# mcgillmrl/prob_mbrl

Hardware: AMD Instinct MI355X
Metric: particle_rollouts_per_sec (higher is better)
Workload: dtype f32 via split fp16 (fwd, 2 pieces) / bf16 (adjoint, 2 pieces) MFMA, fp32 accumulate

## Files before the change

include/pmbrl.h:

```cpp
#ifndef PMBRL_H
#define PMBRL_H

#include <stddef.h>
#include <stdint.h>

#ifdef __cplusplus
extern "C" {
#endif

#define PMBRL_MAX_LAYERS 8
#define PMBRL_MAX_ANGLE 8
#define PMBRL_MAX_TIP 8
#define PMBRL_MAX_DIM 64

#define PMBRL_FLAG_MM_STATES 1
#define PMBRL_FLAG_MM_REWARDS 2
#define PMBRL_FLAG_INFER_NS 4
#define PMBRL_FLAG_FORCE_GENERIC 16
#define PMBRL_FLAG_NO_SHAPED 32
#define PMBRL_FLAG_POL_MASKS_PER_STEP 64
#define PMBRL_FLAG_DYN_MASKS_PER_STEP 128
#define PMBRL_FLAG_GMM_EXACT_NOISE_GRAD 256
#define PMBRL_MAX_COMP 8
#define PMBRL_FLAG_ZMM_PER_STEP 8
// ... 28 lines not shown
  int32_t expand;
  int32_t n_angle;
  int32_t angle_dims[PMBRL_MAX_ANGLE];
  int32_t k;
  float C[PMBRL_MAX_TIP * PMBRL_MAX_DIM];
  float tip_target[PMBRL_MAX_TIP];
  float norm;
  float w;
  float Q[PMBRL_MAX_TIP * PMBRL_MAX_TIP];
  float R[PMBRL_MAX_DIM * PMBRL_MAX_DIM];
} pmbrl_reward;

typedef struct pmbrl_config {
  int32_t B, D, U, H;
  int32_t B_global, row_offset;
  int32_t flags;
  int32_t mm_groups;
  float max_log_std_pol;
  float max_log_std_dyn;
  pmbrl_mlp pol;
  pmbrl_mlp dyn;
  pmbrl_reward reward;
  int32_t rows_per_wg_hint;
  int32_t precision;
  int32_t n_pol_angle;
  int32_t pol_angle_dims[PMBRL_MAX_ANGLE];
  int32_t n_dyn_angle;
  int32_t dyn_angle_dims[PMBRL_MAX_ANGLE];
  int32_t dyn_components;
  int32_t mm_span_rows, mm_span_offset;
  int32_t mm_span_ranks, mm_span_rank;
  int32_t pol_act, dyn_act;
} pmbrl_config;


typedef struct pmbrl_plan pmbrl_plan;

enum {
  PMBRL_INFO_ROWS_PER_WG = 0,
  PMBRL_INFO_N_WG = 1,
  PMBRL_INFO_ROW_TILES = 2,
  PMBRL_INFO_LDS_BYTES = 3,
  PMBRL_INFO_N_POL_PARAMS = 4,
  PMBRL_INFO_N_DYN_PARAMS = 5,
  PMBRL_INFO_DW_SPLITS = 6,
  PMBRL_INFO_MM_MODE = 7,
  PMBRL_INFO_LD = 8,
  PMBRL_INFO_DW_BLOCKS = 9,
  PMBRL_INFO_FAST = 10,
  PMBRL_INFO_STAGES = 11,
  PMBRL_INFO_MM_GRID = 12,
  PMBRL_INFO_PRECISION = 13,
  PMBRL_INFO_DW_PIPE = 14,
  PMBRL_INFO_MM_PARTS = 15,
  PMBRL_INFO_REG = 16,
  PMBRL_INFO_REPLAY = 17,
  PMBRL_INFO_INPLACE = 18,
  PMBRL_INFO_REG_FWD_CALLS = 19,
  PMBRL_INFO_REG_BWD_CALLS = 20,
  PMBRL_INFO_TAIL_CALLS = 21,
  PMBRL_INFO_COUNT = 22
};

const char* pmbrl_last_error(void);
int pmbrl_act_check(int32_t act, int32_t n_hidden);
int pmbrl_version(void);
const char* pmbrl_build_id(void);

typedef struct pmbrl_graph pmbrl_graph;
int pmbrl_graph_capture_begin(void* stream);
int pmbrl_graph_capture_end(void* stream, pmbrl_graph** graph_out);
int pmbrl_graph_launch(pmbrl_graph* graph, void* stream);
int pmbrl_graph_num_nodes(pmbrl_graph* graph, int64_t* n_out);
void pmbrl_graph_destroy(pmbrl_graph* graph);

int pmbrl_plan_create(const pmbrl_config* cfg, int device, pmbrl_plan** out);
void pmbrl_plan_destroy(pmbrl_plan* plan);
size_t pmbrl_plan_workspace_bytes(const pmbrl_plan* plan);
int pmbrl_plan_info(const pmbrl_plan* plan, int32_t* info );
#define PMBRL_SWEEP_REG 4
int pmbrl_plan_sweep_kernel(const pmbrl_plan* plan, int variant, int adjoint, const char** name);
int pmbrl_plan_dw_stream(const pmbrl_plan* plan, int32_t* out );
int pmbrl_plan_dw_head(const pmbrl_plan* plan);

int pmbrl_pack_mask(void* stream, const float* mask_d, int32_t B, int32_t h,
                    int32_t src_ld, uint16_t* bits_d);

int pmbrl_draw_masks(void* stream, int32_t kind, uint64_t seed, uint64_t offset, const float* param_d,
                     int32_t param_len, float temp, int32_t rows, int32_t h, const float* u_d, const float* v_d,
                     uint16_t* bits_d, int32_t aux_row0, int32_t aux_rows, float* u_out_d, float* hard_out_d,
                     float* probs_out_d);

typedef struct pmbrl_inputs {
  const float* x0_d;
  const float* pol_params_d;
  const float* dyn_params_d;
  const float* mx_d;
  const float* iSx_d;
  const float* my_d;
  const float* Sy_d;
  const float* pol_scale_d;
  const float* pol_bias_d;
  const uint16_t* pol_mask_bits_d[PMBRL_MAX_LAYERS];
  const uint16_t* dyn_mask_bits_d[PMBRL_MAX_LAYERS];
  const float* z_pol_d;
  const float* z_dyn_d;
  int64_t z_pol_step_stride;
  int64_t z_dyn_step_stride;
  const float* z_mm_d;
  const float* z_rr_d;
  const float* z_pi_d;
  const float* u_cat_d;
} pmbrl_inputs;

int pmbrl_rollout_fwd(pmbrl_plan* plan, void* stream, void* workspace_d,
                      const pmbrl_inputs* in, float* states_d, float* actions_d,
                      float* rewards_d, int32_t* status_d);

int pmbrl_rollout_bwd(pmbrl_plan* plan, void* stream, void* workspace_d,
                      const pmbrl_inputs* in, const float* states_d,
                      const float* actions_d, const float* rewards_d,
                      const float* grad_rewards_d, const float* grad_states_d,
                      const float* grad_actions_d, float* grad_pol_flat_d,
                      float* grad_x0_d, float* action_grad_norms_d, int32_t* status_d);

int pmbrl_weighted_sum(void* stream, const float* a_d, const float* w_d,
                       int64_t n, float* out_d);
int pmbrl_weighted_sum_steps(void* stream, const float* a_d, const float* w_d,
                             int64_t n_per_step, int32_t n_steps, const int32_t* status_d,
                             float* out_d);

int pmbrl_clip_adam(void* stream, float* params_d, float* grads_d,
                    float* exp_avg_d, float* exp_avg_sq_d, int64_t n,
                    int64_t step, double lr, double beta1, double beta2, double eps,
                    double max_norm, float* norm_out_d);

int pmbrl_clip_adam_guarded(void* stream, float* params_d, float* grads_d,
                            float* exp_avg_d, float* exp_avg_sq_d, int64_t n,
                            int64_t* step_d, double lr, double beta1, double beta2,
                            double eps, double max_norm, float* norm_out_d,
                            const int32_t* status_d, int32_t expect);

typedef struct pmbrl_adam {
  float* params_d;
  float* exp_avg_d;
  float* exp_avg_sq_d;
  int64_t* step_d;
  double lr, beta1, beta2, eps, max_norm;
  float* norm_out_d;
  int32_t expect_steps;
  float* loss_out_d;
} pmbrl_adam;
int pmbrl_plan_set_loss(pmbrl_plan* plan, const float* loss_weights_d, float* loss_out_d);
int pmbrl_rollout_bwd_adam(pmbrl_plan* plan, void* stream, void* workspace_d, const pmbrl_inputs* in,
                           const float* states_d, const float* actions_d, const float* rewards_d,
                           const float* grad_rewards_d, const float* grad_states_d, const float* grad_actions_d,
                           float* grad_pol_flat_d, float* grad_x0_d, float* action_grad_norms_d, int32_t* status_d,
                           const pmbrl_adam* opt);

#define PMBRL_OPT_MAX_GROUPS   8
#define PMBRL_OPT_MAX_SEGMENTS 32
#define PMBRL_OPT_DECOUPLED 1
#define PMBRL_OPT_AMSGRAD   2
#define PMBRL_OPT_MAXIMIZE  4
typedef struct pmbrl_opt_group { double lr, beta1, beta2, eps, weight_decay; int32_t flags; } pmbrl_opt_group;
typedef struct pmbrl_opt_rule {
// ... 148 lines not shown
```

prob_mbrl_amd/_lib.py:

```python
import ctypes as C
import os

_HERE = os.path.dirname(os.path.abspath(__file__))
LIB_PATH = os.environ.get('PMBRL_LIB_PATH', os.path.join(_HERE, 'csrc', 'libpmbrl_hip.so'))

MAX_LAYERS = 8
MAX_ANGLE = 8
MAX_TIP = 8
MAX_DIM = 64
FLAG_MM_STATES, FLAG_MM_REWARDS, FLAG_INFER_NS, FLAG_ZMM_PER_STEP = 1, 2, 4, 8
FLAG_FORCE_GENERIC = 16
FLAG_NO_SHAPED = 32
FLAG_POL_MASKS_PER_STEP, FLAG_DYN_MASKS_PER_STEP = 64, 128
FLAG_GMM_EXACT_NOISE_GRAD = 256
MAX_COMP = 8
REWARD_EXP, REWARD_NEG, REWARD_LEARNED = 0, 1, 2
PREC_F32, PREC_SPLIT, PREC_SPLIT_F16 = 0, 1, 2
ACT_RELU, ACT_TANH, ACT_SILU = 0, 1, 2
DROP_BY_TEMPERATURE, DROP_BERNOULLI = 0, 1
MLP_BWD_MAX_BLOCKS = 256
MLP_BWD_SLAB_BYTES = 64 << 20
(INFO_ROWS_PER_WG, INFO_N_WG, INFO_ROW_TILES, INFO_LDS_BYTES, INFO_N_POL_PARAMS, INFO_N_DYN_PARAMS, INFO_DW_SPLITS,
 INFO_MM_MODE, INFO_LD, INFO_DW_BLOCKS, INFO_FAST, INFO_STAGES, INFO_MM_GRID, INFO_PRECISION, INFO_DW_PIPE, INFO_MM_PARTS,
 INFO_REG, INFO_REPLAY, INFO_INPLACE, INFO_REG_FWD_CALLS, INFO_REG_BWD_CALLS, INFO_TAIL_CALLS, INFO_COUNT) = range(23)
SWEEP_VARIANTS = ('lean', 'ext', 'mm', 'mmg', 'reg')
TIMER_COUNT = 8
TIMER_NAMES = ['pack', 'fwd', 'bwd', 'dw', 'dw_reduce', 'reward']


class MLP(C.Structure):
    _fields_ = [('n_layers', C.c_int32),
                ('dims', C.c_int32 * (MAX_LAYERS + 1)),
                ('keep', C.c_float * MAX_LAYERS)]


class MlpCall(C.Structure):
    _fields_ = [('B', C.c_int32), ('net', MLP), ('max_log_std', C.c_float), ('act', C.c_int32)]


class BnnConfig(C.Structure):
    _fields_ = [('M', C.c_int32), ('N', C.c_int32), ('net', MLP), ('max_log_std', C.c_float),
                ('temperature', C.c_float * MAX_LAYERS), ('reg_scale', C.c_float * MAX_LAYERS),
                ('drop_reg', C.c_float * MAX_LAYERS), ('reg_weight', C.c_float), ('loss_kind', C.c_int32),
                ('n_components', C.c_int32), ('act', C.c_int32),
                ('drop_kind', C.c_int32 * MAX_LAYERS), ('bern_keep', C.c_float * MAX_LAYERS)]


class Reward(C.Structure):
    _fields_ = [('kind', C.c_int32), ('expand', C.c_int32),
                ('n_angle', C.c_int32), ('angle_dims', C.c_int32 * MAX_ANGLE),
                ('k', C.c_int32), ('C', C.c_float * (MAX_TIP * MAX_DIM)),
                ('tip_target', C.c_float * MAX_TIP), ('norm', C.c_float),
                ('w', C.c_float), ('Q', C.c_float * (MAX_TIP * MAX_TIP)),
                ('R', C.c_float * (MAX_DIM * MAX_DIM))]


class Config(C.Structure):
    _fields_ = [('B', C.c_int32), ('D', C.c_int32), ('U', C.c_int32),
                ('H', C.c_int32), ('B_global', C.c_int32),
                ('row_offset', C.c_int32), ('flags', C.c_int32),
                ('mm_groups', C.c_int32), ('max_log_std_pol', C.c_float),
                ('max_log_std_dyn', C.c_float), ('pol', MLP), ('dyn', MLP),
                ('reward', Reward), ('rows_per_wg_hint', C.c_int32), ('precision', C.c_int32),
                ('n_pol_angle', C.c_int32), ('pol_angle_dims', C.c_int32 * MAX_ANGLE),
                ('n_dyn_angle', C.c_int32), ('dyn_angle_dims', C.c_int32 * MAX_ANGLE),
                ('dyn_components', C.c_int32),
                ('mm_span_rows', C.c_int32), ('mm_span_offset', C.c_int32),
                ('mm_span_ranks', C.c_int32), ('mm_span_rank', C.c_int32),
                ('pol_act', C.c_int32), ('dyn_act', C.c_int32)]


COLLECTIVE_FN = C.CFUNCTYPE(C.c_int, C.c_void_p, C.c_void_p, C.c_void_p, C.c_int64)


class Inputs(C.Structure):
    _fields_ = [('x0', C.c_void_p), ('pol_params', C.c_void_p),
                ('dyn_params', C.c_void_p), ('mx', C.c_void_p),
                ('iSx', C.c_void_p), ('my', C.c_void_p), ('Sy', C.c_void_p),
                ('pol_scale', C.c_void_p), ('pol_bias', C.c_void_p),
                ('pol_mask_bits', C.c_void_p * MAX_LAYERS),
                ('dyn_mask_bits', C.c_void_p * MAX_LAYERS),
                ('z_pol', C.c_void_p), ('z_dyn', C.c_void_p),
                ('z_pol_step_stride', C.c_int64), ('z_dyn_step_stride', C.c_int64),
                ('z_mm', C.c_void_p), ('z_rr', C.c_void_p),
                ('z_pi', C.c_void_p), ('u_cat', C.c_void_p)]


EXPORTS = [
    'pmbrl_last_error', 'pmbrl_version', 'pmbrl_build_id', 'pmbrl_plan_create',
    'pmbrl_graph_capture_begin', 'pmbrl_graph_capture_end', 'pmbrl_graph_launch', 'pmbrl_graph_num_nodes', 'pmbrl_graph_destroy',
    'pmbrl_plan_destroy', 'pmbrl_plan_workspace_bytes', 'pmbrl_plan_info', 'pmbrl_plan_sweep_kernel', 'pmbrl_plan_dw_stream',
    'pmbrl_plan_dw_head',
    'pmbrl_pack_mask', 'pmbrl_draw_masks', 'pmbrl_rollout_fwd', 'pmbrl_rollout_bwd', 'pmbrl_rollout_bwd_adam',
    'pmbrl_plan_set_loss',
    'pmbrl_weighted_sum', 'pmbrl_weighted_sum_steps', 'pmbrl_clip_adam', 'pmbrl_clip_adam_guarded', 'pmbrl_debug_linear',
    'pmbrl_plan_set_timing', 'pmbrl_plan_read_timing', 'pmbrl_plan_set_prof', 'pmbrl_plan_set_replay', 'pmbrl_plan_replay_count',
    'pmbrl_mlp_workspace_bytes', 'pmbrl_mlp_forward', 'pmbrl_mlp_grad_input',
    'pmbrl_mlp_backward_workspace_bytes', 'pmbrl_mlp_backward',
    'pmbrl_bnn_plan_create', 'pmbrl_bnn_plan_destroy', 'pmbrl_bnn_plan_workspace_bytes',
    'pmbrl_bnn_plan_n_params', 'pmbrl_bnn_plan_set_unit_keep', 'pmbrl_bnn_loss_grad', 'pmbrl_bnn_loss_grad_ex', 'pmbrl_bnn_train_steps',
    'pmbrl_comm_unique_id', 'pmbrl_comm_init', 'pmbrl_allreduce_sum', 'pmbrl_comm_count', 'pmbrl_comm_destroy',
    'pmbrl_plan_set_comm', 'pmbrl_plan_set_collective',
    'pmbrl_p2p_create', 'pmbrl_p2p_handle', 'pmbrl_p2p_open', 'pmbrl_p2p_allreduce_f32', 'pmbrl_p2p_allreduce_f64',
    'pmbrl_plan_set_p2p', 'pmbrl_p2p_error', 'pmbrl_p2p_destroy', 'pmbrl_plan_set_grad_comm',
    'pmbrl_opt_rule_check', 'pmbrl_clip_adam_rule', 'pmbrl_clip_adam_rule_guarded', 'pmbrl_plan_set_optimizer',
    'pmbrl_bnn_plan_set_optimizer', 'pmbrl_act_check',
]

class Adam(C.Structure):
    _fields_ = [('params_d', C.c_void_p), ('exp_avg_d', C.c_void_p), ('exp_avg_sq_d', C.c_void_p),
                ('step_d', C.c_void_p), ('lr', C.c_double), ('beta1', C.c_double), ('beta2', C.c_double),
                ('eps', C.c_double), ('max_norm', C.c_double), ('norm_out_d', C.c_void_p), ('expect_steps', C.c_int32),
                ('loss_out_d', C.c_void_p)]


OPT_MAX_GROUPS, OPT_MAX_SEGMENTS = 8, 32
OPT_DECOUPLED, OPT_AMSGRAD, OPT_MAXIMIZE = 1, 2, 4


class OptGroup(C.Structure):
    _fields_ = [('lr', C.c_double), ('beta1', C.c_double), ('beta2', C.c_double), ('eps', C.c_double),
                ('weight_decay', C.c_double), ('flags', C.c_int32)]


class OptRule(C.Structure):
    _fields_ = [('n_groups', C.c_int32), ('group', OptGroup * OPT_MAX_GROUPS),
                ('n_segments', C.c_int32), ('seg_end', C.c_int64 * OPT_MAX_SEGMENTS),
                ('seg_group', C.c_int32 * OPT_MAX_SEGMENTS), ('max_exp_avg_sq_d', C.c_void_p)]


_lib = None


def load():
    global _lib
    if _lib is not None:
        return _lib
    if not os.path.exists(LIB_PATH):
        raise RuntimeError(
            'prob_mbrl_amd: %s is missing -- build the HIP extension first '
            '(python -c "import __graft_entry__ as g; g.build()"). There is no '
            'CPU fallback for the rollout hot path.' % LIB_PATH)
    lib = C.CDLL(LIB_PATH)
    vp, i32, i64, f32 = C.c_void_p, C.c_int32, C.c_int64, C.c_float
    lib.pmbrl_last_error.restype = C.c_char_p
    lib.pmbrl_last_error.argtypes = []
    lib.pmbrl_version.restype = C.c_int
    lib.pmbrl_build_id.restype = C.c_char_p
    lib.pmbrl_build_id.argtypes = []
    lib.pmbrl_graph_capture_begin.restype = C.c_int
    lib.pmbrl_graph_capture_begin.argtypes = [vp]
    lib.pmbrl_graph_capture_end.restype = C.c_int
    lib.pmbrl_graph_capture_end.argtypes = [vp, C.POINTER(vp)]
    lib.pmbrl_graph_launch.restype = C.c_int
    lib.pmbrl_graph_launch.argtypes = [vp, vp]
    lib.pmbrl_graph_num_nodes.restype = C.c_int
    lib.pmbrl_graph_num_nodes.argtypes = [vp, C.POINTER(C.c_int64)]
    lib.pmbrl_graph_destroy.restype = None
    lib.pmbrl_graph_destroy.argtypes = [vp]
    lib.pmbrl_plan_create.restype = C.c_int
    lib.pmbrl_plan_create.argtypes = [C.POINTER(Config), C.c_int, C.POINTER(vp)]
    lib.pmbrl_plan_destroy.restype = None
    lib.pmbrl_plan_destroy.argtypes = [vp]
    lib.pmbrl_plan_workspace_bytes.restype = C.c_size_t
    lib.pmbrl_plan_workspace_bytes.argtypes = [vp]
    lib.pmbrl_plan_info.restype = C.c_int
    lib.pmbrl_plan_info.argtypes = [vp, C.POINTER(i32)]
    lib.pmbrl_plan_sweep_kernel.restype = C.c_int
    lib.pmbrl_plan_sweep_kernel.argtypes = [vp, C.c_int, C.c_int, C.POINTER(C.c_char_p)]
    if hasattr(lib, 'pmbrl_plan_dw_stream'):
        lib.pmbrl_plan_dw_stream.restype = C.c_int
        lib.pmbrl_plan_dw_stream.argtypes = [vp, C.POINTER(i32)]
    if hasattr(lib, 'pmbrl_plan_dw_head'):
        lib.pmbrl_plan_dw_head.restype = C.c_int
        lib.pmbrl_plan_dw_head.argtypes = [vp]
    lib.pmbrl_pack_mask.restype = C.c_int
    lib.pmbrl_pack_mask.argtypes = [vp, vp, i32, i32, i32, vp]
    lib.pmbrl_rollout_fwd.restype = C.c_int
    lib.pmbrl_rollout_fwd.argtypes = [vp, vp, vp, C.POINTER(Inputs), vp, vp, vp, vp]
    lib.pmbrl_rollout_bwd.restype = C.c_int
    lib.pmbrl_rollout_bwd.argtypes = [vp, vp, vp, C.POINTER(Inputs), vp, vp, vp,
                                      vp, vp, vp, vp, vp, vp, vp]
    lib.pmbrl_weighted_sum.restype = C.c_int
    lib.pmbrl_weighted_sum.argtypes = [vp, vp, vp, i64, vp]
    lib.pmbrl_weighted_sum_steps.restype = C.c_int
    lib.pmbrl_weighted_sum_steps.argtypes = [vp, vp, vp, i64, i32, vp, vp]
    lib.pmbrl_clip_adam.restype = C.c_int
    f64 = C.c_double
    lib.pmbrl_clip_adam.argtypes = [vp, vp, vp, vp, vp, i64, i64, f64, f64, f64,
                                    f64, f64, vp]
    lib.pmbrl_clip_adam_guarded.restype = C.c_int
    lib.pmbrl_clip_adam_guarded.argtypes = [vp, vp, vp, vp, vp, i64, vp, f64, f64, f64, f64, f64, vp, vp, i32]
    lib.pmbrl_mlp_workspace_bytes.restype = C.c_size_t
    lib.pmbrl_mlp_workspace_bytes.argtypes = [C.POINTER(MlpCall)]
    lib.pmbrl_mlp_forward.restype = C.c_int
    lib.pmbrl_mlp_forward.argtypes = [vp, C.POINTER(MlpCall), vp, vp, vp, C.POINTER(vp)] + [vp] * 10
    lib.pmbrl_mlp_grad_input.restype = C.c_int
    lib.pmbrl_mlp_grad_input.argtypes = [vp, C.POINTER(MlpCall), vp, vp, vp, C.POINTER(vp)] + [vp] * 11
    lib.pmbrl_mlp_backward_workspace_bytes.restype = C.c_size_t
    lib.pmbrl_mlp_backward_workspace_bytes.argtypes = [C.POINTER(MlpCall)]
    lib.pmbrl_mlp_backward.restype = C.c_int
    lib.pmbrl_mlp_backward.argtypes = [vp, C.POINTER(MlpCall), vp, vp, vp, C.POINTER(vp)] + [vp] * 12
    lib.pmbrl_bnn_plan_create.restype = C.c_int
    lib.pmbrl_bnn_plan_create.argtypes = [C.POINTER(BnnConfig), C.c_int, C.POINTER(vp)]
    lib.pmbrl_bnn_plan_destroy.restype = None
    lib.pmbrl_bnn_plan_destroy.argtypes = [vp]
    lib.pmbrl_bnn_plan_workspace_bytes.restype = C.c_size_t
    lib.pmbrl_bnn_plan_workspace_bytes.argtypes = [vp]
    lib.pmbrl_bnn_plan_n_params.restype = C.c_int64
    lib.pmbrl_bnn_plan_n_params.argtypes = [vp]
    lib.pmbrl_bnn_plan_set_unit_keep.restype = C.c_int
    lib.pmbrl_bnn_plan_set_unit_keep.argtypes = [vp, i32, C.POINTER(f32), i32]
    lib.pmbrl_bnn_loss_grad.restype = C.c_int
    lib.pmbrl_bnn_loss_grad.argtypes = [vp] * 11
    lib.pmbrl_bnn_loss_grad_ex.restype = C.c_int
    lib.pmbrl_bnn_loss_grad_ex.argtypes = [vp] * 13 + [i32]
    lib.pmbrl_bnn_train_steps.restype = C.c_int
    lib.pmbrl_bnn_train_steps.argtypes = ([vp] * 6 + [i32] + [vp] * 4 + [C.c_double] * 4 + [C.c_uint64] * 2 + [vp] * 4)
    lib.pmbrl_debug_linear.restype = C.c_int
    lib.pmbrl_debug_linear.argtypes = [vp, vp, vp, vp, i32, i32, i32, i32, vp, vp]
    lib.pmbrl_plan_set_replay.restype = C.c_int
    lib.pmbrl_plan_set_replay.argtypes = [vp, C.c_int]
    lib.pmbrl_plan_replay_count.restype = C.c_int
    lib.pmbrl_plan_replay_count.argtypes = [vp, C.POINTER(C.c_int64)]
    lib.pmbrl_plan_set_timing.restype = C.c_int
    lib.pmbrl_plan_set_timing.argtypes = [vp, C.c_int]
    lib.pmbrl_plan_read_timing.restype = C.c_int
    lib.pmbrl_plan_read_timing.argtypes = [vp, C.POINTER(C.c_float)]
    lib.pmbrl_plan_set_prof.restype = C.c_int
    lib.pmbrl_plan_set_prof.argtypes = [vp, vp, vp]
    lib.pmbrl_comm_unique_id.restype = C.c_int
    lib.pmbrl_comm_unique_id.argtypes = [vp]
    lib.pmbrl_comm_init.restype = C.c_int
    lib.pmbrl_comm_init.argtypes = [vp, i32, i32, i32, C.POINTER(vp)]
    lib.pmbrl_allreduce_sum.restype = C.c_int
    lib.pmbrl_allreduce_sum.argtypes = [vp, vp, vp, i64]
    lib.pmbrl_plan_set_loss.restype = C.c_int
    lib.pmbrl_plan_set_loss.argtypes = [vp, vp, vp]
    lib.pmbrl_rollout_bwd_adam.restype = C.c_int
    lib.pmbrl_rollout_bwd_adam.argtypes = [vp, vp, vp, C.POINTER(Inputs)] + [vp] * 10 + [C.POINTER(Adam)]
    lib.pmbrl_draw_masks.restype = C.c_int
    lib.pmbrl_draw_masks.argtypes = [vp, i32, C.c_uint64, C.c_uint64, vp, i32, C.c_float, i32, i32, vp, vp, vp, i32, i32, vp, vp, vp]
    lib.pmbrl_comm_count.restype = C.c_int
    lib.pmbrl_comm_count.argtypes = [vp, C.POINTER(i32)]
    lib.pmbrl_comm_destroy.restype = None
    lib.pmbrl_comm_destroy.argtypes = [vp]
    lib.pmbrl_plan_set_comm.restype = C.c_int
    lib.pmbrl_plan_set_comm.argtypes = [vp, vp]
    lib.pmbrl_p2p_create.restype = C.c_int
    lib.pmbrl_p2p_create.argtypes = [i32, i32, i32, i64, C.POINTER(vp)]
    lib.pmbrl_p2p_handle.restype = C.c_int
    lib.pmbrl_p2p_handle.argtypes = [vp, vp]
    lib.pmbrl_p2p_open.restype = C.c_int
    lib.pmbrl_p2p_open.argtypes = [vp, i32, vp]
    for fn in (lib.pmbrl_p2p_allreduce_f32, lib.pmbrl_p2p_allreduce_f64):
        fn.restype = C.c_int
        fn.argtypes = [vp, vp, vp, i64]
    lib.pmbrl_plan_set_p2p.restype = C.c_int
# ... 39 lines not shown
```

prob_mbrl_amd/csrc/pmbrl.hip:

```cpp
#include <hip/hip_runtime.h>
#include <math.h>
#include <stdio.h>
#include <string.h>

#include <algorithm>
#include <memory>
#include <string>
#include <vector>

#include "pmbrl_host.h"
#include "pmbrl_mm.h"
#include "pmbrl_rollout.h"
#include "pmbrl_mmx.h"
#include "pmbrl_mm_wide.h"
#include "pmbrl_fast.h"
#include "pmbrl_reward.h"

static thread_local std::string g_err;
int pm_fail(int code, const std::string& msg) {
  g_err = msg;
  return code;
}

extern "C" const char* pmbrl_last_error(void) { return g_err.c_str(); }
// ... 293 lines not shown
  return why ? fail(-2, why) : 0;
}

static int net_plan(const pmbrl_mlp& m, int act, NetPlan& n, int in_expect, int out_expect,
                    const char* name) {
  if (m.n_layers < 1 || m.n_layers > PM_MAXL)
    return fail(-2, std::string(name) + ": n_layers out of range");
  n.nl = m.n_layers;
  size_t off = 0;
  for (int i = 0; i <= n.nl; ++i) {
    if (m.dims[i] < 1 || m.dims[i] > 4096) return fail(-2, std::string(name) + ": bad layer width");
    n.dim[i] = m.dims[i];
    n.nt[i] = (m.dims[i] + 15) / 16;
  }
  if (n.dim[0] != in_expect || n.dim[n.nl] != out_expect)
    return fail(-2, std::string(name) + ": input/output width does not match D/U");
  if (const char* why = pm_act_refusal(act, n.nl - 1)) return fail(-2, std::string(name) + ": " + why);
  n.act = pm_act_layers(act, n.nl - 1);
  for (int l = 0; l < n.nl; ++l) {
    n.keep[l] = (l < n.nl - 1) ? m.keep[l] : 1.f;
    if (l < n.nl - 1 && !(n.keep[l] > 0.f)) return fail(-2, std::string(name) + ": keep must be > 0");
    n.w_off[l] = off;
    off += (size_t)n.dim[l + 1] * n.dim[l];
    n.b_off[l] = off;
    off += n.dim[l + 1];
  }
  n.n_params = off;
  return 0;
}

#define PM_INST(RT, CA, CB, VAR, D, U, LD, NL, NT, TREE) \
  {reinterpret_cast<const void*>(&pm_rollout_fwd<RT>), reinterpret_cast<const void*>(&pm_rollout_bwd<RT>)},
static const PmInst general_f32_fns[] = {PM_GENERAL_F32_INSTANCES};
#undef PM_INST
static_assert(sizeof(general_f32_fns) / sizeof(general_f32_fns[0]) == pm_general_f32_n, "one kernel pair per key");

static constexpr size_t PM_LDS_CAP = 160 * 1024;

static bool env_set(const char* name) { return getenv(name) != nullptr; }
static bool env_on(const char* name) {
  const char* e = getenv(name);
  return !(e && atoi(e) == 0);
}
static PlanSwitches read_switches() {
  PlanSwitches s{};
  s.mm_perstep = env_set("PMBRL_MM_PERSTEP");
  s.mm_mode2 = env_set("PMBRL_MM_MODE2");
  s.mm_no_batch = env_set("PMBRL_MM_NO_BATCH");
  s.dw_no_wide = env_set("PMBRL_DW_NO_WIDE");
  s.reg_debug = env_set("PMBRL_REG_DEBUG");
  s.lds_tiles = env_on("PMBRL_LDS_TILES");
  s.mm_xch = env_on("PMBRL_MM_XCH");
  s.mm_tree = env_on("PMBRL_MM_TREE");
  s.reg = env_on("PMBRL_REG");
  s.reg_mm = env_on("PMBRL_REG_MM");
  s.reg_tree = env_on("PMBRL_REG_TREE");
  s.reg_bwd = env_on("PMBRL_REG_BWD");
  s.fuse_loss = env_on("PMBRL_FUSE_LOSS");
  s.ztab_merge = env_on("PMBRL_ZTAB_MERGE");
  s.wide = env_on("PMBRL_WIDE");
  if (const char* e = getenv("PMBRL_MM_PARTS")) { s.mm_parts_set = true; s.mm_parts = atoi(e); }
  s.replay = 1;
  if (const char* e = getenv("PMBRL_REPLAY")) s.replay = std::max(0, std::min(2, atoi(e)));
  if (const char* e = getenv("PMBRL_DW_PIPE")) {
    s.dw_pipe_off = !strcmp(e, "off");
    s.dw_pipe_ranges = e[0] >= '0' && e[0] <= '9';
    for (const char* q = e; s.dw_pipe_ranges && *q;) {
      const int v = atoi(q);
      if (v > 0) s.dw_pipe.push_back(v);
      while (*q && *q != ',') ++q;
      if (*q == ',') ++q;
    }
  }
  s.dw_head = -1;
  if (const char* e = getenv("PMBRL_DW_HEAD")) s.dw_head = !strcmp(e, "on") ? 1 : (!strcmp(e, "off") ? 0 : -1);
  if (const char* e = getenv("PMBRL_DW_STREAM")) {
    s.dw_stream_off = !strcmp(e, "off");
    s.dw_stream_set = e[0] >= '0' && e[0] <= '9';
    if (s.dw_stream_set) {
      s.dw_stream_steps = atoi(e);
      if (const char* q = strchr(e, ',')) s.dw_stream_wgs = std::max(0, atoi(q + 1));
    }
  }
  return s;
}

static int plan_nets(pmbrl_plan* p) {
  const pmbrl_config& c = p->cfg;
  if (c.n_pol_angle < 0 || c.n_pol_angle > PMBRL_MAX_ANGLE || c.n_dyn_angle < 0 || c.n_dyn_angle > PMBRL_MAX_ANGLE)
    return fail(-2, "n_pol_angle / n_dyn_angle out of range");
  if (c.dyn_components < 0 || c.dyn_components > PMBRL_MAX_COMP)
    return fail(-2, "dyn_components out of range (<= PMBRL_MAX_COMP)");
  const bool gmm = c.dyn_components > 1;
  if (c.reward.kind != PMBRL_REWARD_EXP && c.reward.kind != PMBRL_REWARD_NEG && c.reward.kind != PMBRL_REWARD_LEARNED)
    return fail(-2, "unknown reward kind");
  p->learned = c.reward.kind == PMBRL_REWARD_LEARNED;
  if (p->learned && c.mm_span_rows > 0)
    return fail(-2, "learned reward head: not offered with moment-matching groups spread over ranks (mm_span_rows > 0)");
  if (p->learned && c.D + 1 > PMBRL_MAX_DIM) return fail(-2, "learned reward head: D + 1 exceeds PMBRL_MAX_DIM");
  if (p->learned && gmm && c.dyn.n_layers >= 1 && c.dyn.n_layers <= PM_MAXL &&
      c.dyn.dims[c.dyn.n_layers] != (2 * (c.D + 1) + 1) * c.dyn_components + 1)
    return fail(-2, "learned reward head with the mixture head: the density has D + 1 dimensions, a dynamics head "
                    "(2 (D + 1) + 1) dyn_components + 1 wide");
  int rc = net_plan(c.pol, c.pol_act, p->pol, c.D + c.n_pol_angle, 2 * c.U, "policy");
  if (rc == 0)
    rc = net_plan(c.dyn, c.dyn_act, p->dyn, c.D + c.U + c.n_dyn_angle,
                  gmm ? (2 * (c.D + p->learned) + 1) * c.dyn_components + 1 : 2 * (c.D + p->learned), "dynamics");
  p->act = rc == 0 && (p->pol.act != 0 || p->dyn.act != 0);
  return rc;
}

struct LayoutCalc {
  const pmbrl_plan* p;
  int maxnt;
  bool gsplit;
  bool want_split;
  bool rt4_split;
  int ld_generic() const { return gsplit ? (maxnt * 16 + 31) / 32 * 32 + 16 : maxnt * 16 + 8; }
  int prec(int RT) const {
    if (!p->fast) return gsplit ? (int)PMBRL_PREC_SPLIT_F16 : 0;
    return (want_split && (RT <= 2 || rt4_split)) ? (int)p->cfg.precision : 0;
  }
  long stream_work(int m, int kdiv) const {
    long w = 0;
    for (const NetPlan* n : {&p->pol, &p->dyn})
      for (int l = 1; l <= n->nl - 2; ++l) {
        const int ki = (n->nt[l] + kdiv - 1) / kdiv, ko = (n->nt[l + 1] + kdiv - 1) / kdiv;
        w += (long)n->nt[l + 1] * ((ki + m - 1) / m * m) + (long)n->nt[l] * ((ko + m - 1) / m * m);
      }
    return w;
  }
  StagePair stages(int RT) const {
    const int pr = prec(RT);
    return pm_inst_best_stages(pm_fast_keys(pr), pr && !p->fast ? std::min(RT, 2) : RT,
                               [&](int m) { return stream_work(m, pr ? 2 : 1); });
  }
  int ldb(int RT) const {
    if (!prec(RT)) return 0;
    if (!p->fast) return ld_generic();
    const StagePair sp = stages(RT);
    const int m = sp.ca + sp.cb;
    return ((maxnt + 1) / 2 + m - 1) / m * m * 32 + 16;
  }
  int ld(int RT) const {
    if (!p->fast) return ld_generic();
    if (prec(RT))
      return ((prec(RT) == PMBRL_PREC_SPLIT_F16 ? 2 : 3) * ldb(RT) / 2 + 3) / 4 * 4;
    const StagePair sp = stages(RT);
    const int m = sp.ca + sp.cb;
    return (maxnt + m - 1) / m * m * 16 + 8;
  }
  PmFastMap fast_map(int RT, int mmd, int parts = 1) const {
    const pmbrl_config& c = p->cfg;
    const int mw = parts > 1 ? 1 : (mmd && p->M <= 16 * RT) ? std::min(PF_NW, std::max(1, 16 * RT / p->M)) : PF_NW;
    return pm_fast_map(16 * RT, ld(RT), c.D, c.U, RT, p->pol.nt, p->pol.nl, p->dyn.nt, p->dyn.nl, mmd, prec(RT), mw,
                       parts > 1 ? (parts > 8 ? 16 : p->M) : 0, parts > 1 ? c.H : 0);
  }
  size_t lds(int RT, int mmd, int parts = 1, bool inplace = false) const {
    const pmbrl_config& c = p->cfg;
    if (p->fast) return fast_map(RT, mmd, parts).total * sizeof(float);
    return pm_lds_map(0, 16 * RT, ld(RT), c.D, c.U, RT, mmd, inplace).total * sizeof(float);
  }
};

static int plan_groups(pmbrl_plan* p, LayoutCalc& L, int cus) {
  const pmbrl_config& c = p->cfg;
// ... 534 lines not shown
}

extern "C" int pmbrl_plan_set_replay(pmbrl_plan* p, int on) {
  if (!p || on < 0 || on > 2) return fail(-1, "bad argument");
  p->replay = on;
  for (int k = 0; k < 2; ++k) { replay_drop(p, k); p->rp[k].dead = 0; }
  return 0;
}

extern "C" int pmbrl_plan_replay_count(const pmbrl_plan* p, int64_t* n_out) {
  if (!p || !n_out) return fail(-1, "null argument");
  for (int k = 0; k < 2; ++k) n_out[k] = p->rp[k].launches;
  return 0;
}

extern "C" int pmbrl_plan_set_prof(pmbrl_plan* p, long long* fwd_d, long long* bwd_d) {
  if (!p) return fail(-1, "null argument");
  p->prof_fwd = fwd_d;
  p->prof_bwd = bwd_d;
  return 0;
}

extern "C" int pmbrl_plan_set_timing(pmbrl_plan* p, int on) {
  if (!p) return fail(-1, "null argument");
  if (on && !p->ev[0][0]) {
    for (int i = 0; i < PMBRL_TIMER_COUNT; ++i)
      for (int j = 0; j < 2; ++j) HIPCHK(hipEventCreate(&p->ev[i][j]));
  }
  p->timing = on ? 1 : 0;
  for (int i = 0; i < PMBRL_TIMER_COUNT; ++i) p->ev_set[i] = false;
  return 0;
}

extern "C" int pmbrl_plan_read_timing(pmbrl_plan* p, float* ms) {
  if (!p || !ms) return fail(-1, "null argument");
  for (int i = 0; i < PMBRL_TIMER_COUNT; ++i) {
    ms[i] = -1.f;
    if (p->timing && p->ev_set[i]) {
      HIPCHK(hipEventSynchronize(p->ev[i][1]));
      HIPCHK(hipEventElapsedTime(&ms[i], p->ev[i][0], p->ev[i][1]));
    }
  }
  return 0;
}

extern "C" void pmbrl_plan_destroy(pmbrl_plan* p) {
  if (!p) return;
  if (p->ev[0][0])
    for (int i = 0; i < PMBRL_TIMER_COUNT; ++i)
      for (int j = 0; j < 2; ++j) (void)hipEventDestroy(p->ev[i][j]);
  for (int k = 0; k < 2; ++k) replay_drop(p, k);
  if (p->cap_stream) (void)hipStreamDestroy(p->cap_stream);
  if (p->rew_d) (void)hipFree(p->rew_d);
  if (p->wflag_d) (void)hipFree(p->wflag_d);
  if (p->ang_d) (void)hipFree(p->ang_d);
  pm_dw_plan_destroy(p);
  if (p->tail_buf_d) (void)hipFree(p->tail_buf_d);
  delete p;
}

extern "C" int pmbrl_plan_sweep_kernel(const pmbrl_plan* p, int variant, int adjoint, const char** name) {
  if (!p || !name) return fail(-1, "null argument");
  PmInst k{};
  if (variant == PMBRL_SWEEP_REG) k = p->reg ? p->reg_k[0] : k;
  else if (!p->fast) k = p->sweep[0];
  else if (variant >= 0 && variant < PF_VAR_COUNT) k = p->sweep[variant];
  else return fail(-1, "variant out of range");
  const void* f = adjoint ? k.bwd : k.fwd;
  *name = f ? hipKernelNameRefByPtr(f, nullptr) : "";
  if (!*name) *name = "";
  return 0;
}

extern "C" size_t pmbrl_plan_workspace_bytes(const pmbrl_plan* p) { return p ? p->ws_bytes : 0; }

extern "C" int pmbrl_plan_dw_stream(const pmbrl_plan* p, int32_t* out) {
  if (!p || !out) return fail(-1, "null argument");
  out[0] = p->dw.st_on ? p->cfg.H - p->dw.st_cut : -1;
  out[1] = p->dw.st_on ? p->dw.st_wgs : 0;
  return 0;
}

extern "C" int pmbrl_plan_dw_head(const pmbrl_plan* p) { return p && p->dw.st_on && p->dw.st_head ? 1 : 0; }

extern "C" int pmbrl_plan_info(const pmbrl_plan* p, int32_t* info) {
  if (!p || !info) return fail(-1, "null argument");
  memset(info, 0, sizeof(int32_t) * PMBRL_INFO_COUNT);
  info[PMBRL_INFO_ROWS_PER_WG] = p->rows_per_wg;
  info[PMBRL_INFO_N_WG] = p->nwg;
  info[PMBRL_INFO_ROW_TILES] = p->RT;
  info[PMBRL_INFO_LDS_BYTES] = (int32_t)p->lds_bytes;
  info[PMBRL_INFO_N_POL_PARAMS] = (int32_t)p->pol.n_params;
  info[PMBRL_INFO_N_DYN_PARAMS] = (int32_t)p->dyn.n_params;
  info[PMBRL_INFO_DW_SPLITS] = p->dw.args.nsplit;
  info[PMBRL_INFO_MM_MODE] = p->mm_mode;
  info[PMBRL_INFO_LD] = p->LD;
  info[PMBRL_INFO_DW_BLOCKS] = p->dw.n_blocks();
  info[PMBRL_INFO_FAST] = p->fast;
  info[PMBRL_INFO_STAGES] = p->CA * 16 + p->CB;
  info[PMBRL_INFO_MM_GRID] = p->mm_grid;
  info[PMBRL_INFO_PRECISION] = p->prec;
  info[PMBRL_INFO_DW_PIPE] = p->dw.pipe_K;
  info[PMBRL_INFO_MM_PARTS] = p->mm_parts;
  info[PMBRL_INFO_REG] = p->reg;
  info[PMBRL_INFO_REPLAY] = replay_wanted(p) ? 1 : 0;
  info[PMBRL_INFO_INPLACE] = p->inplace;
  info[PMBRL_INFO_REG_FWD_CALLS] = p->reg_calls[0];
  info[PMBRL_INFO_REG_BWD_CALLS] = p->reg_calls[1];
  info[PMBRL_INFO_TAIL_CALLS] = p->tail_calls;
  return 0;
}


static void fill_net(const NetPlan& n, char* ws, const uint16_t* const* masks, NetDev& d) {
  d.nl = n.nl;
  for (int i = 0; i <= n.nl; ++i) {
    d.dim[i] = n.dim[i];
    d.nt[i] = n.nt[i];
  }
  for (int l = 0; l < n.nl; ++l) {
    d.keep[l] = n.keep[l];
    d.inv_keep[l] = 1.f / n.keep[l];
    d.wf[l] = reinterpret_cast<const float*>(ws + n.wf[l]);
    d.wb[l] = reinterpret_cast<const float*>(ws + n.wb[l]);
    d.bias[l] = reinterpret_cast<const float*>(ws + n.bias[l]);
    d.mask[l] = (l < n.nl - 1) ? masks[l] : nullptr;
    d.abits[l] = (l < n.nl - 1) ? reinterpret_cast<uint16_t*>(ws + n.abits[l]) : nullptr;
  }
}

static int fill_args(const pmbrl_plan* p, void* workspace, const pmbrl_inputs* in, RolloutArgs& A) {
  const pmbrl_config& c = p->cfg;
  char* ws = static_cast<char*>(workspace);
  memset(&A, 0, sizeof(A));
  A.B = c.B; A.D = c.D; A.U = c.U; A.H = c.H;
  A.Bg = c.B_global; A.row_off = c.row_offset; A.flags = c.flags;
  A.pol_acts = p->pol.act; A.dyn_acts = p->dyn.act;
  A.G = p->G; A.M = p->M; A.mm_mode = p->mm_mode;
  A.t0 = 0; A.t1 = c.H;
  A.rows_per_wg = p->rows_per_wg; A.nwg = p->nwg; A.Rw = 16 * p->RT; A.LD = p->LD; A.LDB = p->LDB;
  A.mls_pol = c.max_log_std_pol; A.mls_dyn = c.max_log_std_dyn;
  for (int l = 0; l < p->pol.nl - 1; ++l)
    if (!in->pol_mask_bits_d[l]) return fail(-1, "missing policy mask bits");
  for (int l = 0; l < p->dyn.nl - 1; ++l)
    if (!in->dyn_mask_bits_d[l]) return fail(-1, "missing dynamics mask bits");
  fill_net(p->pol, ws, in->pol_mask_bits_d, A.pol);
  fill_net(p->dyn, ws, in->dyn_mask_bits_d, A.dyn);
  A.rew = p->rew_d;
  A.ang = p->ang_d;
  A.x0 = in->x0_d; A.mx = in->mx_d; A.iSx = in->iSx_d; A.my = in->my_d; A.Sy = in->Sy_d;
  A.pscale = in->pol_scale_d; A.pbias = in->pol_bias_d;
  A.zpol = in->z_pol_d; A.zdyn = in->z_dyn_d; A.zmm = in->z_mm_d; A.zrr = in->z_rr_d;
  A.zpol_ss = in->z_pol_step_stride; A.zdyn_ss = in->z_dyn_step_stride;
  if (!A.x0 || !A.mx || !A.iSx || !A.my || !A.Sy || !A.pscale || !A.pbias || !A.zpol || !A.zdyn)
    return fail(-1, "null input pointer");
  if ((c.flags & PMBRL_FLAG_MM_STATES) && !A.zmm) return fail(-1, "mm_states needs z_mm");
  if ((c.flags & PMBRL_FLAG_MM_REWARDS) && !A.zrr) return fail(-1, "mm_rewards needs z_rr");
  for (int l = 0; l < p->pol.nl; ++l) {
    A.actT[l] = reinterpret_cast<float*>(ws + p->off_actT[l]);
    A.gT[l] = reinterpret_cast<float*>(ws + p->off_gT[l]);
  }
  A.Tp = reinterpret_cast<float*>(ws + p->off_Tp);
  A.Td = reinterpret_cast<float*>(ws + p->off_Td);
  A.gmm_n = p->cfg.dyn_components > 1 ? p->cfg.dyn_components : 0;
  A.zpi = A.ucat = A.zdyn_grad = nullptr;
  A.gmm_k = nullptr;
// ... 530 lines not shown
static int bwd_sweep_external(pmbrl_plan* p, const BwdCall& C, RolloutArgs A, float* grt) {
  hipStream_t s = C.stream;
  char* ws = static_cast<char*>(C.workspace);
  const size_t smem = pm_mm_kernel_doubles(p->cfg.D) * sizeof(double);
  HIPCHK(hipMemsetAsync(A.gx_carry, 0, (size_t)p->cfg.B * p->cfg.D * sizeof(float), s));
  RolloutArgs Am = A;
  Am.flags &= ~PMBRL_FLAG_MM_REWARDS;
  A.gx_from_carry = 1;
  for (int t = p->cfg.H - 1; t >= 0; --t) {
    if (p->mm_wide) {
      hipLaunchKernelGGL(pm_mmw_bwd_kernel, dim3(p->G), dim3(PM_MMW_NT), pm_mmw_lds_bytes(p->M, p->cfg.D, true), s, Am, t,
                         reinterpret_cast<const double*>(ws + p->off_mmfac));
    } else if (!p->span) {
      hipLaunchKernelGGL(pm_mm_bwd_kernel, dim3(p->G), dim3(PM_MM_NW * 64), smem, s, Am, t, grt);
    } else if (p->cfg.flags & PMBRL_FLAG_MM_STATES) {
      if (int rc = mmx_bwd(p, ws, Am, false, t, nullptr, s)) return rc;
    }
    A.t0 = t; A.t1 = t + 1;
    launch_bwd_rt(p, A, s);
  }
  return 0;
}

static int bwd_dw(pmbrl_plan* p, const BwdCall& C, const DwArgs& W, bool piped) {
  ScopedTimer tm(p, PMBRL_TIMER_DW, C.stream);
  if (!piped) {
    pm_dw_launch(p, W, C.stream, W.st_on ? p->dw.pipe_ev[1] : nullptr);
    return 0;
  }
  HIPCHK(hipEventRecord(p->dw.pipe_ev[p->dw.pipe_K - 1], p->dw.pipe_stream));
  HIPCHK(hipStreamWaitEvent(C.stream, p->dw.pipe_ev[p->dw.pipe_K - 1], 0));
  pm_dw_launch_range(p, W, p->dw.pipe_K - 1, C.stream);
  return 0;
}

static bool bwd_streamed(const pmbrl_plan* p, const BwdCall& C, bool reg_bwd) {
  return p->dw.st_on && reg_bwd && sweep_form(p) == SweepForm::Whole && p->dw.pipe_K <= 1 && !p->prof_bwd && !bwd_tail(p, C);
}
static int rollout_bwd(pmbrl_plan* p, const BwdCall& C, const RolloutArgs& A0, bool reg_bwd) {
  hipStream_t s = C.stream;
  RolloutArgs A = A0;
  if (int rc = check_bwd(p, C, reg_bwd)) return rc;
  const pmbrl_adam* opt = C.opt;
  const bool tail = bwd_tail(p, C);
  float* const xb = p->tail_buf_d;
  if (tail)
    if (int rc = bwd_agree_horizon(p, C)) return rc;
  if (p->reg && !reg_bwd) bwd_convert_family(p, C);
  float* grt = reinterpret_cast<float*>(static_cast<char*>(C.workspace) + p->off_grt);
  if (int rc = bwd_reward_adjoint(p, C, A, grt)) return rc;
  const SweepForm form = sweep_form(p);
  const bool piped = form == SweepForm::Whole && p->dw.pipe_K > 1 && !p->prof_bwd;
  const bool streamed = bwd_streamed(p, C, reg_bwd);
  const DwArgs W = pm_dw_call_args(p, C.workspace, C.status, A, reg_bwd, streamed);
  {
    ScopedTimer tm(p, PMBRL_TIMER_BWD, s);
    static const int whole[1] = {0};
    int rc = 0;
    switch (form) {
      case SweepForm::Barrier: rc = bwd_sweep_barrier(p, C, A); break;
      case SweepForm::StepInSweep: rc = bwd_sweep_steps(p, C, A); break;
      case SweepForm::Whole: rc = bwd_sweep_whole(p, C, A, W, reg_bwd, piped ? p->dw.pipe_K : 1, piped ? p->dw.pipe_lo : whole); break;
      case SweepForm::StepExternal: rc = bwd_sweep_external(p, C, A, grt); break;
    }
    if (rc) return rc;
  }
  if (int rc = bwd_dw(p, C, W, piped)) return rc;
  const int n = (int)p->pol.n_params;
  const int expect = expect_steps(p, opt);
  const bool part_ok = opt && !piped && (n + 255) / 256 <= PM_NORM_MAXB;
  const bool norm_fused = part_ok && !tail;
  const bool loss_fused = part_ok && opt->loss_out_d && p->sw.fuse_loss;
  const int n_loss_part = loss_fused ? (n + 255) / 256 : 0;
  float* const red_out = tail ? xb : C.grad_pol_flat;
  {
    ScopedTimer tm(p, PMBRL_TIMER_DW_REDUCE, s);
    if (piped)
      pm_dw_reduce_launch(s, W.part, p->dw.pipe_rows, n, W.part_stride, red_out, (const int*)nullptr, 0, 1);
    else
      pm_dw_reduce_launch(s, W.part, p->dw.args.nsplit, n, W.part_stride, red_out, (const int*)C.status, W.chunks_per_step,
                          W.chunks_per_split, norm_fused ? 1 : 0, (const int*)C.status, expect,
                          opt ? reinterpret_cast<long long*>(opt->step_d) : (long long*)nullptr,
                          loss_fused ? C.rewards : (const float*)nullptr, C.grad_rewards, (long long)p->cfg.H * p->cfg.B,
                          (long long)p->cfg.B, W.own_lo, W.own_hi, W.st_wgs);
  }
  if (opt && opt->loss_out_d && !loss_fused)
    launch_weighted_sum(s, C.rewards, C.grad_rewards, (long long)p->cfg.H * p->cfg.B, tail ? xb + n : opt->loss_out_d, C.status,
                        p->cfg.B);
  HIPCHK(hipGetLastError());
  if (!opt) return 0;
  if (tail) {
    pm_tail_pack_launch(s, xb, n, n_loss_part, opt->loss_out_d && !loss_fused ? 1 : 0, C.status, p->tail_err_d);
    if (int rc = tail_allreduce(p, s, xb, (int64_t)n + 2)) return rc;
    pm_tail_finish_launch(s, xb, C.grad_pol_flat, n, C.status, expect, reinterpret_cast<long long*>(opt->step_d), p->tail_err_d);
    HIPCHK(hipGetLastError());
  }
  AdamStep S;
  S.params = opt->params_d; S.grads = C.grad_pol_flat; S.exp_avg = opt->exp_avg_d; S.exp_avg_sq = opt->exp_avg_sq_d; S.n = n;
  S.step_d = opt->step_d; S.status = C.status; S.expect = expect;
  S.max_norm = opt->max_norm; S.norm_out = opt->norm_out_d;
  S.norm_done = tail || norm_fused;
  S.loss_out = tail || loss_fused ? opt->loss_out_d : nullptr;
  S.n_loss_part = tail ? (opt->loss_out_d ? 1 : 0) : n_loss_part;
  S.lr = opt->lr; S.beta1 = opt->beta1; S.beta2 = opt->beta2; S.eps = opt->eps;
  S.rule = p->has_opt_rule ? &p->opt_rule : nullptr;
  return pm_adam_launch(s, S);
}

static ReplayKey bwd_key(const pmbrl_plan* p, const BwdCall& C, bool reg_bwd) {
  const pmbrl_adam* opt = C.opt;
  ReplayKey K;
  K.val(C.stream); K.val(C.workspace); K.add(C.in, sizeof(*C.in));
  K.val(C.states); K.val(C.actions); K.val(C.rewards); K.val(C.grad_rewards); K.val(C.grad_states); K.val(C.grad_actions);
  K.val(C.grad_pol_flat); K.val(C.grad_x0); K.val(C.action_grad_norms); K.val(C.status);
  const int has_opt = opt ? 1 : 0;
  K.val(has_opt);
  if (opt) {
    K.val(opt->params_d); K.val(opt->exp_avg_d); K.val(opt->exp_avg_sq_d); K.val(opt->step_d);
    K.val(opt->lr); K.val(opt->beta1); K.val(opt->beta2); K.val(opt->eps); K.val(opt->max_norm);
    K.val(opt->norm_out_d); K.val(opt->expect_steps);
    K.val(p->has_opt_rule);
    if (p->has_opt_rule) {
      const pmbrl_opt_rule& R = p->opt_rule;
      K.val(R.n_groups); K.val(R.n_segments); K.val(R.max_exp_avg_sq_d);
      for (int g = 0; g < R.n_groups; ++g) {
        const pmbrl_opt_group& G = R.group[g];
        K.val(G.lr); K.val(G.beta1); K.val(G.beta2); K.val(G.eps); K.val(G.weight_decay); K.val(G.flags);
      }
      for (int q = 0; q < R.n_segments; ++q) { K.val(R.seg_end[q]); K.val(R.seg_group[q]); }
    }
  }
  if (bwd_tail(p, C)) {
    K.val(p->grad_comm); K.val(p->tail_buf_d); K.val(opt->loss_out_d);
  }
  K.val(p->old_pack_stale); K.val(p->abits_packed);
  const int g1_rebuilt = reg_bwd ? 1 : 0;
  K.val(g1_rebuilt);
  const int streamed = bwd_streamed(p, C, reg_bwd) ? 1 : 0;
  K.val(streamed);
  const int head = streamed && p->dw.st_head ? 1 : 0;
  K.val(head);
  return K;
}

static int rollout_bwd_replay(pmbrl_plan* p, const BwdCall& C) {
  if (!p || !C.workspace || !C.in || !C.states || !C.actions || !C.rewards || !C.grad_rewards || !C.grad_pol_flat)
    return fail(-1, "null argument");
  HIPCHK(hipSetDevice(p->device));
  RolloutArgs A;
  if (int rc = bwd_args(p, C, A)) return rc;
  const bool reg_bwd = pm_reg_can_run(p, A, false);
  const bool tail = bwd_tail(p, C);
  if (tail) ++p->tail_calls;
  if (tail && p->grad_p2p) {
    if (p->rp[1].exec || p->rp[1].seen) replay_drop(p, 1);
    return rollout_bwd(p, C, A, reg_bwd);
  }
  return replay_call(p, 1, bwd_key(p, C, reg_bwd), C.stream, [&](hipStream_t on) {
    BwdCall Con = C;
    Con.stream = on;
    return rollout_bwd(p, Con, A, reg_bwd);
  });
}

extern "C" int pmbrl_rollout_bwd(pmbrl_plan* p, void* stream, void* workspace, const pmbrl_inputs* in,
                                 const float* states_d, const float* actions_d,
                                 const float* rewards_d, const float* grad_rewards_d,
                                 const float* grad_states_d, const float* grad_actions_d,
                                 float* grad_pol_flat_d, float* grad_x0_d,
                                 float* action_grad_norms_d, int32_t* status_d) {
  return rollout_bwd_replay(p, BwdCall{(hipStream_t)stream, workspace, in, states_d, actions_d, rewards_d, grad_rewards_d,
                                       grad_states_d, grad_actions_d, grad_pol_flat_d, grad_x0_d, action_grad_norms_d,
                                       status_d, nullptr});
}

extern "C" int pmbrl_rollout_bwd_adam(pmbrl_plan* p, void* stream, void* workspace, const pmbrl_inputs* in,
                                      const float* states_d, const float* actions_d,
                                      const float* rewards_d, const float* grad_rewards_d,
                                      const float* grad_states_d, const float* grad_actions_d,
                                      float* grad_pol_flat_d, float* grad_x0_d,
                                      float* action_grad_norms_d, int32_t* status_d, const pmbrl_adam* opt) {
  if (!opt || !status_d || !opt->params_d || !opt->exp_avg_d || !opt->exp_avg_sq_d || !opt->step_d)
    return fail(-1, "null argument");
  return rollout_bwd_replay(p, BwdCall{(hipStream_t)stream, workspace, in, states_d, actions_d, rewards_d, grad_rewards_d,
                                       grad_states_d, grad_actions_d, grad_pol_flat_d, grad_x0_d, action_grad_norms_d,
                                       status_d, opt});
}

template <int RT>
__global__ __launch_bounds__(PM_NT, 1) void pm_debug_linear_kernel(const float* x, const float* wf,
                                                                  const float* bias, int R, int K,
                                                                  int O, int LD, int narrow,
                                                                  float* y) {
  extern __shared__ __attribute__((aligned(16))) float smem[];
  const int tid = threadIdx.x, lane = tid & 63, wid = tid >> 6;
  constexpr int RR = 16 * RT;
  float* X = smem;
  float* Y = X + RR * LD;
  float* part = pm_part_alias_ok(RR, LD, RT) ? nullptr : Y + RR * LD;
  const int n_kb = (K + 15) / 16, n_ot = (O + 15) / 16;
  for (int i = tid; i < RR * LD; i += PM_NT) {
    const int r = i / LD, k = i - r * LD;
    X[i] = (r < R && k < K) ? x[(size_t)r * K + k] : 0.f;
  }
  __syncthreads();
  if (narrow) {
    gemm_narrow<RT>(wf, n_ot, n_kb, bias, X, Y, LD, part, wid, lane, tid);
  } else {
    EpiPlain e{bias, Y, LD, lane};
    gemm_tiles<RT>(wf, n_ot, n_kb, X, LD, wid, lane, e);
    __syncthreads();
  }
  for (int i = tid; i < R * O; i += PM_NT) {
    const int r = i / O, o = i - r * O;
    y[i] = Y[r * LD + o];
  }
}

extern "C" int pmbrl_debug_linear(void* stream, const float* x_d, const float* W_d, const float* b_d,
                                  int32_t R, int32_t K, int32_t O, int32_t transpose_w, float* y_d,
                                  float* scratch_d) {
  if (R < 1 || R > 64 || K < 1 || O < 1) return fail(-1, "bad argument");
  hipStream_t s = (hipStream_t)stream;
  const int n_kb = (K + 15) / 16, n_ot = (O + 15) / 16;
// ... 39 lines not shown
```

prob_mbrl_amd/csrc/pmbrl_dw.h:

```cpp
#pragma once
#include <stdint.h>

#include "pmbrl.h"

#define PM_MAXL PMBRL_MAX_LAYERS

#define PM_DW_NW 8
#define PM_DW_NT (PM_DW_NW * 64)
#define PM_DW_TM 4
#define PM_DW_TN 7
#define PM_DW_MAXBLK 256
#define PM_DW_TN_S 4

struct DwBlock {
  int16_t layer, ot0, it0, n_ot, n_it, pad;
};
struct DwUnit {
  int16_t layer, m0, n0, pad;
};
#define PM_DWW_TM 128
#define PM_DWW_TN 128
#define PM_DWW_LDK 40
#define PM_DWW_STAGE ((PM_DWW_TM + PM_DWW_TN) * 2 * PM_DWW_LDK)
#define PM_DWW_LDS_BYTES (2 * PM_DWW_STAGE * 2)

struct DwArgs {
  int nl, nsplit, n_chunks, chunks_per_split;
  int RT, Rw, n_params;
  int part_stride;
  int dim[PM_MAXL + 1], nt[PM_MAXL + 1];
  int w_off[PM_MAXL], b_off[PM_MAXL];
  const float* actT[PM_MAXL];
  const float* gT[PM_MAXL];
  const int* nvalid;
  int chunks_per_step;
  const DwBlock* blocks;
  int wave_first[PM_DW_NW + 1];
  float* part;
  int split_prec;
  int pipe;
  int pipe_k;
  int c_begin, c_end;
  int rows_before;
  const unsigned* rc_abits;
  const float* rc_head;
  float rc_inv_keep;
  int rc_D, rc_U;
  int st_on;
  int st_cut, st_wgs;
  const unsigned long long* st_pub;
  unsigned st_tag;
  int* st_fail;
  int own_lo, own_hi;
  int st_head;
};
static_assert(sizeof(DwArgs) == 472, "DwArgs is a kernel argument: its layout does not move");
#define PM_DWH_LDS_BYTES ((2 * 16 * 16 + PM_DW_NW * 64 * 12) * 4)

#define PM_DWP_TM 256
#define PM_DWP_TN 256
#define PM_DWL_NT 13
```

prob_mbrl_amd/csrc/pmbrl_dw.hip:

```cpp
#include <hip/hip_runtime.h>

#include <algorithm>
#include <cassert>
#include <vector>

#include "pmbrl_host.h"
#include "pmbrl_dw_kernels.h"

static int pm_dw_set_attr(const DwPlan& D) {
  const bool layer = D.layer13 >= 0, pre = D.pre_mask != 0, units = D.unit_k != DwKernel::None;
  const struct { bool on; const void* fn; int bytes; } K[] = {
      {layer, reinterpret_cast<const void*>(&pm_dw_layer_kernel), PM_DWL_LDS_BYTES},
      {layer, reinterpret_cast<const void*>(&pm_dw_layer_rc_kernel), PM_DWL_LDS_BYTES},
      {layer, reinterpret_cast<const void*>(&pm_dw_layer_st_kernel), PM_DWL_LDS_BYTES + PM_DWH_LDS_BYTES},
      {layer, reinterpret_cast<const void*>(&pm_dw_layer_rcb_kernel), PM_DWL_LDS_BYTES},
      {pre, reinterpret_cast<const void*>(&pm_dw_narrow_pre_kernel<1>), PM_DWP_LDS_BYTES},
      {pre, reinterpret_cast<const void*>(&pm_dw_narrow_pre_kernel<2>), PM_DWP_LDS_BYTES},
      {units, reinterpret_cast<const void*>(&pm_dw_wide_kernel), PM_DWW_LDS_BYTES},
      {D.unit_k == DwKernel::WidePre, reinterpret_cast<const void*>(&pm_dw_wide_pre_kernel), PM_DWP_LDS_BYTES}};
  for (const auto& k : K)
    if (k.on) HIPCHK(hipFuncSetAttribute(k.fn, hipFuncAttributeMaxDynamicSharedMemorySize, k.bytes));
  return 0;
}

hipError_t pm_dw_upload_blocks(const std::vector<DwBlock>& blocks, DwBlock** out) {
  *out = nullptr;
  hipError_t e = hipMalloc(out, std::max<size_t>(1, blocks.size()) * sizeof(DwBlock));
  if (e == hipSuccess && !blocks.empty()) e = hipMemcpy(*out, blocks.data(), blocks.size() * sizeof(DwBlock), hipMemcpyHostToDevice);
  if (e != hipSuccess && *out) { (void)hipFree(*out); *out = nullptr; }
  return e;
}
void pm_dw_bind_blocks(DwArgs& W, const DwBlock* blocks_d, const int* wave_first) {
  W.blocks = blocks_d;
  for (int w = 0; w <= PM_DW_NW; ++w) W.wave_first[w] = wave_first[w];
}

int pm_dw_plan_create(pmbrl_plan* p, int cus) {
  DwShape S{};
  S.nl = p->pol.nl;
  for (int i = 0; i <= S.nl; ++i) { S.nt[i] = p->pol.nt[i]; S.dim[i] = p->pol.dim[i]; }
  for (int l = 0; l < S.nl; ++l) { S.w_off[l] = (int)p->pol.w_off[l]; S.b_off[l] = (int)p->pol.b_off[l]; }
  S.n_params = (int)p->pol.n_params; S.dyn_n_params = (int)p->dyn.n_params;
  S.prec = p->prec; S.RT = p->RT; S.fast = p->fast; S.inplace = p->inplace; S.nwg = p->nwg;
  S.H = p->cfg.H; S.U = p->cfg.U; S.cus = cus;
  S.whole = sweep_form(p) == SweepForm::Whole;
  S.mm_parts = p->mm_parts; S.reg = p->reg; S.reg_mm = p->reg_mm; S.reg_bwd = p->sw.reg_bwd;
  S.sw = p->sw;
  DwPlan& D = p->dw;
  pm_dw_plan(S, D);
  if (!D.units.empty()) {
    HIPCHK(hipMalloc(&D.units_d, D.units.size() * sizeof(DwUnit)));
    HIPCHK(hipMemcpy(D.units_d, D.units.data(), D.units.size() * sizeof(DwUnit), hipMemcpyHostToDevice));
  }
  if (int rc = pm_dw_set_attr(D)) return rc;
  DwBlock* blocks_d = nullptr;
  HIPCHK(pm_dw_upload_blocks(D.blocks, &blocks_d));
  D.args.blocks = blocks_d;
  if (D.pipe_K > 1 || D.st_on) {
    HIPCHK(hipStreamCreateWithFlags(&D.pipe_stream, hipStreamNonBlocking));
    for (int k = 0; k < std::max(D.pipe_K, D.st_on ? 2 : 0); ++k)
      HIPCHK(hipEventCreateWithFlags(&D.pipe_ev[k], hipEventDisableTiming));
  }
  if (D.st_head && pm_dw_upload_blocks(D.blocks_nh, &D.blocks_nh_d) != hipSuccess) {
    (void)hipGetLastError();
    D.st_head = 0;
    D.table_nh_k = DwKernel::None;
  }
  return 0;
}
void pm_dw_plan_destroy(pmbrl_plan* p) {
  DwPlan& D = p->dw;
  if (D.args.blocks) (void)hipFree(const_cast<DwBlock*>(D.args.blocks));
  if (D.blocks_nh_d) (void)hipFree(D.blocks_nh_d);
  if (D.units_d) (void)hipFree(D.units_d);
  if (D.pipe_stream) (void)hipStreamDestroy(D.pipe_stream);
  for (int k = 0; k < PM_PIPE_MAX; ++k)
    if (D.pipe_ev[k]) (void)hipEventDestroy(D.pipe_ev[k]);
}

DwArgs pm_dw_call_args(const pmbrl_plan* p, void* workspace, int32_t* status, const RolloutArgs& A, bool rebuilt, bool streamed) {
  const DwPlan& D = p->dw;
  DwArgs W = D.args;
  if (streamed) {
    W.st_on = 1;
    W.st_cut = D.st_cut;
    W.st_wgs = D.st_wgs;
    W.st_pub = reinterpret_cast<const unsigned long long*>(static_cast<char*>(workspace) + D.off_pub);
    W.st_tag = ((++D.pub_gen) << 12) + 1u;
    W.st_fail = status ? status + 1 : nullptr;
    if (W.st_cut == 0) {
      const int l = D.layer13;
      if (W.b_off[l] == W.w_off[l] + W.dim[l + 1] * W.dim[l]) {
        W.own_lo = W.w_off[l];
        W.own_hi = W.b_off[l] + W.dim[l + 1];
      }
      if (D.st_head) {
        W.st_head = 1;
        W.own_hi = W.b_off[l + 1] + W.dim[l + 2];
        pm_dw_bind_blocks(W, D.blocks_nh_d, D.wave_first_nh);
      }
    }
  }
  for (int l = 0; l < p->pol.nl; ++l) { W.actT[l] = A.actT[l]; W.gT[l] = A.gT[l]; }
  W.part = reinterpret_cast<float*>(static_cast<char*>(workspace) + D.off_part);
  W.nvalid = status;
  assert(!rebuilt || (W.RT == 1 && D.layer13 == PM_REG_DW_LAYER));
  assert(!streamed || rebuilt);
  if (rebuilt) {
    pm_reg_dw_rebuild_args(p, static_cast<char*>(workspace), W);
    W.rc_inv_keep = A.pol.inv_keep[1];
  }
  return W;
}
static DwArgs dw_range_args(const DwPlan& D, const DwArgs& W, int k, int H) {
  DwArgs Wk = W;
  const int cps = W.chunks_per_step;
  Wk.pipe = 1;
  Wk.pipe_k = k;
  Wk.nsplit = k + 1 == D.pipe_K ? D.pipe_rows : D.pipe_grid;
  Wk.rows_before = D.pipe_grid;
  Wk.c_begin = D.pipe_lo[k] * cps;
  Wk.c_end = (k ? D.pipe_lo[k - 1] : H) * cps;
  Wk.chunks_per_split = (Wk.c_end - Wk.c_begin + Wk.nsplit - 1) / Wk.nsplit;
  if (W.split_prec) Wk.chunks_per_split = (Wk.chunks_per_split + 1) & ~1;
  return Wk;
}
void pm_dw_launch(const pmbrl_plan* p, const DwArgs& W, hipStream_t s, hipEvent_t after) {
  const DwPlan& D = p->dw;
  const int n_units = (int)D.units.size();
  const dim3 rows(W.nsplit), units((W.nsplit + 7) / 8 * 8 * n_units);
  switch (W.st_head ? D.table_nh_k : D.table_k) {
    case DwKernel::Block: hipLaunchKernelGGL(pm_dw_kernel, rows, dim3(PM_DW_NT), 0, s, W); break;
    case DwKernel::BlockSplit: hipLaunchKernelGGL(pm_dw_kernel_s, rows, dim3(PM_DW_NT), 0, s, W); break;
    case DwKernel::BlockRing: hipLaunchKernelGGL(pm_dw_kernel_nh, rows, dim3(PM_DW_NT), 0, s, W); break;
    default: break;
  }
  for (int l = 0; l < W.nl; ++l) {
    const int g_wide = D.narrow[l] == 1 ? 1 : 0;
    if (D.layer_k[l] == DwKernel::NarrowPre1)
      hipLaunchKernelGGL(pm_dw_narrow_pre_kernel<1>, rows, dim3(PM_DWP_NT), PM_DWP_LDS_BYTES, s, W, l, g_wide);
    else if (D.layer_k[l] == DwKernel::NarrowPre2)
      hipLaunchKernelGGL(pm_dw_narrow_pre_kernel<2>, rows, dim3(PM_DWP_NT), PM_DWP_LDS_BYTES, s, W, l, g_wide);
  }
  if (D.unit_k == DwKernel::WidePre)
    hipLaunchKernelGGL(pm_dw_wide_pre_kernel, units, dim3(PM_DWP_NT), PM_DWP_LDS_BYTES, s, W, D.units_d, n_units);
  else if (D.unit_k == DwKernel::Wide)
    hipLaunchKernelGGL(pm_dw_wide_kernel, units, dim3(PM_DW_NT), PM_DWW_LDS_BYTES, s, W, D.units_d, n_units);
  if (after) (void)hipStreamWaitEvent(s, after, 0);
  if (W.st_on && W.st_cut == 0) return;
  if (D.layer13 < 0) return;
  if (W.st_on) hipLaunchKernelGGL(pm_dw_layer_rcb_kernel, rows, dim3(PM_DW_NT), PM_DWL_LDS_BYTES, s, W, D.layer13);
  else if (W.rc_abits) hipLaunchKernelGGL(pm_dw_layer_rc_kernel, rows, dim3(PM_DW_NT), PM_DWL_LDS_BYTES, s, W, D.layer13);
  else hipLaunchKernelGGL(pm_dw_layer_kernel, rows, dim3(PM_DW_NT), PM_DWL_LDS_BYTES, s, W, D.layer13);
}
void pm_dw_launch_range(const pmbrl_plan* p, const DwArgs& W, int k, hipStream_t s) { pm_dw_launch(p, dw_range_args(p->dw, W, k, p->cfg.H), s); }
void pm_dw_stream_launch(const pmbrl_plan* p, const DwArgs& W, hipStream_t s) {
  assert(W.st_on && W.rc_abits);
  hipLaunchKernelGGL(pm_dw_layer_st_kernel, dim3(W.st_wgs), dim3(PM_DW_NT), PM_DWL_LDS_BYTES + PM_DWH_LDS_BYTES, s, W,
                     p->dw.layer13);
}
void pm_dw_blocks_launch(const DwArgs& W, hipStream_t s) {
  hipLaunchKernelGGL(pm_dw_kernel, dim3(W.nsplit), dim3(PM_DW_NT), 0, s, W);
}
```

prob_mbrl_amd/csrc/pmbrl_dw_kernels.h:

```cpp
#pragma once
#include "pmbrl_dw.h"
#include "pmbrl_split.h"
#include "pmbrl_reg_head.h"

#include <utility>
#include <type_traits>
template <class F, int... I>
__device__ __forceinline__ void pr_for_dw_impl(F&& f, std::integer_sequence<int, I...>) { (f(std::integral_constant<int, I>{}), ...); }
template <int N, class F>
__device__ __forceinline__ void pr_for_dw(F&& f) { pr_for_dw_impl(static_cast<F&&>(f), std::make_integer_sequence<int, N>{}); }
typedef unsigned pr_u32x4_dw __attribute__((ext_vector_type(4)));
typedef unsigned long long pr_u64x2_dw __attribute__((ext_vector_type(2)));

struct PmTrue { static constexpr bool value = true; };
struct PmFalse { static constexpr bool value = false; };

struct DwRange {
  int c_lo, c_hi;
  bool add;
  bool zero;
};

__device__ __forceinline__ void pm_dw_ld(f32x4& d, unsigned voff, const float* sbase) {
#ifdef PM_EXP_DW_NOLOAD
// ... 1043 lines not shown
};
typedef __attribute__((address_space(1))) const unsigned long long pm_dw_gu64;
struct PmDwRcSt : PmDwRc {
  unsigned long long gr[2][2][2];
  const unsigned long long* gp;
  unsigned want;
  int gblk;
  bool gsecond, dead;
  int ab_wv[2];
  unsigned lane_;

  __device__ __forceinline__ void init_st(const DwArgs& A, int wid, int lane) {
    gblk = 2 * A.rc_U * 16;
    dead = false;
    lane_ = (unsigned)lane;
#pragma unroll
    for (int i = 0; i < 2; ++i) {
      const int tr = (i == 0 || wid + 8 < PM_DWL_NT) ? wid + 8 * i : wid;
      ab_wv[i] = tr == PR_XT ? pr_xwave(0) : (tr & (PR_NW - 1));
    }
  }
  __device__ __forceinline__ void load() {
#pragma unroll
    for (int h = 0; h < 2; ++h) {
      pm_dw_gu64* q = (pm_dw_gu64*)gp + ((h == 1 && gsecond) ? gblk : 0);
#pragma unroll
      for (int s = 0; s < 2; ++s) {
        gr[h][s][0] = __hip_atomic_load(q + hoff_m[s], __ATOMIC_RELAXED, __HIP_MEMORY_SCOPE_AGENT);
        gr[h][s][1] = __hip_atomic_load(q + (gblk >> 1) + hoff_m[s], __ATOMIC_RELAXED, __HIP_MEMORY_SCOPE_AGENT);
      }
    }
  }
  __device__ __forceinline__ void fetch_st(const DwArgs& A, int c, bool second, int t) {
    gp = A.st_pub + (size_t)c * gblk;
    want = A.st_tag + (unsigned)t;
    gsecond = second;
    load();
#pragma unroll
    for (int h = 0; h < 2; ++h) {
      const unsigned* ap = A.rc_abits + (size_t)(c + h) * (PR_NW * 64);
#pragma unroll
      for (int i = 0; i < 2; ++i) abw[h][i] = (h == 0 || second) ? ap[ab_wv[i] * 64 + (int)lane_] : 0u;
    }
  }
  __device__ __forceinline__ void settle(const DwArgs& A, int lane) {
    for (int spins = 0;;) {
      bool here = true;
#pragma unroll
      for (int h = 0; h < 2; ++h)
#pragma unroll
        for (int s = 0; s < 2; ++s) {
          const bool live = (h == 0 || gsecond) && hok[s];
          here = here && (!live || ((unsigned)(gr[h][s][0] >> 32) == want && (unsigned)(gr[h][s][1] >> 32) == want));
        }
      if (__all(here) || dead) break;
      for (;;) {
        if (++spins > (1 << 19)) {
          dead = true;
          if (lane == 0 && A.st_fail) atomicMax(A.st_fail, 1);
          break;
        }
        __builtin_amdgcn_s_sleep(32);
        const unsigned long long g1 = __hip_atomic_load((pm_dw_gu64*)gp, __ATOMIC_RELAXED, __HIP_MEMORY_SCOPE_AGENT);
        if ((unsigned)(g1 >> 32) == want) break;
      }
      if (dead) break;
      load();
    }
#pragma unroll
    for (int h = 0; h < 2; ++h)
#pragma unroll
      for (int s = 0; s < 2; ++s) {
        const bool live = (h == 0 || gsecond) && hok[s];
        hgm[h][s] = live ? __uint_as_float((unsigned)gr[h][s][0]) : 0.f;
        hgl[h][s] = live ? __uint_as_float((unsigned)gr[h][s][1]) : 0.f;
      }
  }
};
#define PM_DWH_TAB (2 * 16 * 16)
#define PM_DWH_WAVE (64 * 12)
static_assert(PM_DWH_LDS_BYTES == (PM_DWH_TAB + PM_DW_NW * PM_DWH_WAVE) * 4, "the head's LDS");
#define PM_DWL_RT (ST == 1 ? 1 : A.RT)
#define PM_DWL_RW (ST == 1 ? 16 : A.Rw)
template <bool RC, int ST = 0>
__device__ __forceinline__ void pm_dw_layer_body(const DwArgs& A, int l) {
  static_assert(RC || ST == 0, "the streamed form rebuilds its operand");
  extern __shared__ __attribute__((aligned(16))) unsigned short dww_lds[];
  const int tid = threadIdx.x, lane = tid & 63;
  const int wid = __builtin_amdgcn_readfirstlane(tid >> 6);
  const int row = blockIdx.x;
  DwRange R;
  int st_steps = 0, k_lo = 0, k_hi = 0;
  if constexpr (ST == 1) {
    const DwStream S = pm_dw_stream(A);
    if (!S.any || row >= S.nc) return;
    st_steps = S.steps;
    k_lo = (int)((long long)row * A.chunks_per_step / S.nc);
    k_hi = (int)((long long)(row + 1) * A.chunks_per_step / S.nc);
    R.add = false;
    R.zero = k_lo >= k_hi;
    R.c_lo = R.c_hi = 0;
    if (A.st_cut == 0) {
      const int O_ = A.dim[l + 1], K_ = A.dim[l];
      const int a_lo = (A.own_lo + 3) & ~3, a_hi = A.own_hi & ~3;
      for (int r = S.nc + row; r < S.rows; r += S.nc) {
        float* pz = A.part + (size_t)r * A.part_stride;
        if (a_lo < a_hi) {
          if (tid < a_lo - A.own_lo) pz[A.own_lo + tid] = 0.f;
          if (tid < A.own_hi - a_hi) pz[a_hi + tid] = 0.f;
        } else {
          for (int e = tid; e < O_ * K_; e += PM_DW_NT) pz[A.w_off[l] + e] = 0.f;
          for (int e = tid; e < O_; e += PM_DW_NT) pz[A.b_off[l] + e] = 0.f;
        }
      }
    }
  } else if constexpr (ST == 2) {
    if (!pm_dw_range_st(A, row, R)) return;
  } else {
    if (!pm_dw_range(A, row, R)) return;
  }
  const int Fo16 = A.nt[l + 1] * 16, Fi16 = A.nt[l] * 16;
  const int O = A.dim[l + 1], K = A.dim[l];
  float* part = A.part + (size_t)row * A.part_stride;
  const int g = lane >> 4, c16 = lane & 15;
  if (R.zero) {
    for (int e = tid; e < O * K; e += PM_DW_NT) part[A.w_off[l] + e] = 0.f;
    for (int e = tid; e < O; e += PM_DW_NT) part[A.b_off[l] + e] = 0.f;
    if constexpr (ST == 1) {
      if (A.st_head) {
        const int O2 = A.dim[l + 2];
        for (int e = tid; e < O2 * O; e += PM_DW_NT) part[A.w_off[l + 1] + e] = 0.f;
        for (int e = tid; e < O2; e += PM_DW_NT) part[A.b_off[l + 1] + e] = 0.f;
      }
    }
    return;
  }
  const float* gbase = A.gT[l];
  const float* abase = A.actT[l];
  const size_t gblk = (size_t)Fo16 * PM_DWL_RW, ablk = (size_t)Fi16 * PM_DWL_RW;
  f32x4 rb[PM_DWL_Q];
  float* const hd_tab = reinterpret_cast<float*>(dww_lds) + PM_DWL_LDS_BYTES / 4;
  const unsigned hd_lo = (unsigned)(c16 * 16 + 4 * g);
  float* const hd_acc = hd_tab + PM_DWH_TAB + wid * PM_DWH_WAVE;
  if constexpr (ST == 1) {
    if (A.st_head) {
      for (int e = tid; e < PM_DWH_TAB; e += PM_DW_NT) hd_tab[e] = 0.f;
      for (int e = lane; e < PM_DWH_WAVE; e += 64) hd_acc[e] = 0.f;
      __syncthreads();
    }
  }
  std::conditional_t<RC, PmDwNone, PmDwFetched> cl;
  std::conditional_t<RC, std::conditional_t<ST == 1, PmDwRcSt, PmDwRc>, PmDwNone> rc;
  if constexpr (ST == 1) rc.init_st(A, wid, lane);
  if constexpr (RC) rc.init(A, l, wid, lane);
  else {
#pragma unroll
    for (int j = 0; j < PM_DWL_Q; ++j) cl.bs[j] = 0.f;
  }
  auto fetch1 = [&](f32x4& dst, const float* base, size_t blk, int F16, int idx, int c, bool second) {
    const int f = idx >> 3, kq = idx & 7;
    const float* p;
    bool live = f < F16;
    if (PM_DWL_RT >= 2) {
      const int b = c / PM_DWL_RT, rt = c - b * PM_DWL_RT;
      p = base + (size_t)b * blk + (size_t)f * PM_DWL_RW + rt * 16 + kq * 4;
    } else {
      p = base + (size_t)(c + (kq >> 2)) * blk + (size_t)f * 16 + (kq & 3) * 4;
      live = live && (kq < 4 || second);
    }
    dst = live ? *reinterpret_cast<const f32x4*>(p) : f32x4{0.f, 0.f, 0.f, 0.f};
  };
  const bool pow2 = (PM_DWL_RT & (PM_DWL_RT - 1)) == 0;
  const int rt_sh = PM_DWL_RT >= 4 ? 2 : (PM_DWL_RT >= 2 ? 1 : 0);
  unsigned offB[PM_DWL_Q];
#pragma unroll
  for (int j = 0; j < PM_DWL_Q; ++j) {
    const int idx = tid + PM_DW_NT * j, f = idx >> 3, kq = idx & 7;
    const int fa = min(f, Fo16 - 1), fb = min(f, Fi16 - 1);
    if (PM_DWL_RT >= 2) {
      if constexpr (!RC) cl.offA[j] = (unsigned)(fa * PM_DWL_RW + kq * 4);
      offB[j] = (unsigned)(fb * PM_DWL_RW + kq * 4);
// ... 29 lines not shown
    }
#pragma unroll
    for (int j = 0; j < PM_DWL_Q; ++j) {
      const int idx = tid + PM_DW_NT * j;
      if constexpr (!RC) fetch1(cl.ra[j], gbase, gblk, Fo16, idx, c, second);
      fetch1(rb[j], abase, ablk, Fi16, idx, c, second);
    }
  };
  f32x4 ha[2][2];
  auto head_load = [&](int c, bool second) {
    if constexpr (ST == 1) {
      const size_t hblk = (size_t)Fo16 * 16;
#pragma unroll
      for (int h = 0; h < 2; ++h) {
        const float* ph = A.actT[l + 1] + (size_t)(c + ((h == 1 && second) ? 1 : 0)) * hblk;
#pragma unroll
        for (int i = 0; i < 2; ++i) {
          const int tr = min(wid + 8 * i, A.nt[l + 1] - 1);
          ha[h][i] = *reinterpret_cast<const f32x4*>(ph + tr * 256 + hd_lo);
          if (h == 1 && !second) ha[h][i] = f32x4{0.f, 0.f, 0.f, 0.f};
        }
      }
    }
  };
  auto head_mfma = [&]() {
    if constexpr (ST == 1) {
      float* const tm = hd_tab + ((2 * g - A.rc_D) * 16 + c16);
      float* const tl = tm + A.rc_U * 16;
#pragma unroll
      for (int h = 0; h < 2; ++h)
#pragma unroll
        for (int s = 0; s < 2; ++s)
          if (rc.hok[s]) {
            tm[h * 256 + s * 16] = rc.hgm[h][s];
            tl[h * 256 + s * 16] = rc.hgl[h][s];
          }
      __builtin_amdgcn_fence(__ATOMIC_RELEASE, "wavefront");
      __builtin_amdgcn_wave_barrier();
      __builtin_amdgcn_fence(__ATOMIC_ACQUIRE, "wavefront");
      f32x4 hg[2], hacc[2];
#pragma unroll
      for (int h = 0; h < 2; ++h) hg[h] = *reinterpret_cast<const f32x4*>(hd_tab + h * 256 + hd_lo);
#pragma unroll
      for (int i = 0; i < 2; ++i) hacc[i] = *reinterpret_cast<const f32x4*>(hd_acc + lane * 12 + 4 * i);
      float hb = hd_acc[lane * 12 + 8];
      const bool two2 = wid + 8 < A.nt[l + 1];
#pragma unroll
      for (int h = 0; h < 2; ++h) {
#pragma unroll
        for (int kk = 0; kk < 4; ++kk) {
          hacc[0] = mfma4(hg[h][kk], ha[h][0][kk], hacc[0]);
          if (two2) hacc[1] = mfma4(hg[h][kk], ha[h][1][kk], hacc[1]);
        }
        hb += (hg[h][0] + hg[h][1]) + (hg[h][2] + hg[h][3]);
      }
#pragma unroll
      for (int i = 0; i < 2; ++i) *reinterpret_cast<f32x4*>(hd_acc + lane * 12 + 4 * i) = hacc[i];
      hd_acc[lane * 12 + 8] = hb;
    }
  };
  auto put = [&](unsigned short* plane, int f, int kq, const f32x4& v) {
    const unsigned h0 = pm_pk_bf16(v[0], v[1]), h1 = pm_pk_bf16(v[2], v[3]);
    const unsigned l0 = pm_pk_bf16(v[0] - pm_bf_lo(h0), v[1] - pm_bf_hi(h0));
    const unsigned l1 = pm_pk_bf16(v[2] - pm_bf_lo(h1), v[3] - pm_bf_hi(h1));
    unsigned short* q = plane + f * PM_DWW_LDK + kq * 4;
    *reinterpret_cast<uint2*>(q) = uint2{h0, h1};
    *reinterpret_cast<uint2*>(q + PM_DWL_F * PM_DWW_LDK) = uint2{l0, l1};
  };
  auto stage = [&](int st, int c = 0, bool second = false) {
    unsigned short* sa = dww_lds + st * PM_DWL_STAGE;
    unsigned short* sb = sa + 2 * PM_DWL_F * PM_DWW_LDK;
#pragma unroll
    for (int j = 0; j < PM_DWL_Q; ++j) {
      const int idx = tid + PM_DW_NT * j;
      if (idx < PM_DWL_F * 8) {
        if constexpr (!RC) put(sa, idx >> 3, idx & 7, cl.ra[j]);
        put(sb, idx >> 3, idx & 7, rb[j]);
        if constexpr (!RC) cl.bs[j] += (cl.ra[j][0] + cl.ra[j][1]) + (cl.ra[j][2] + cl.ra[j][3]);
      }
    }
    if constexpr (ST == 1) {
      __builtin_amdgcn_sched_barrier(0);
      if (A.st_head) head_load(c, second);
      rc.settle(A, lane);
      if (A.st_head) head_mfma();
      __builtin_amdgcn_sched_barrier(0);
    }
    if constexpr (RC) rc.stage(sa, A.rc_inv_keep, lane);
  };
  f32x4 acc[2][PM_DWL_NT];
#pragma unroll
  for (int i = 0; i < 2; ++i)
#pragma unroll
    for (int j = 0; j < PM_DWL_NT; ++j) acc[i][j] = f32x4{0.f, 0.f, 0.f, 0.f};
  const bool two = wid + 8 < PM_DWL_NT;
  auto mfmas = [&](int st) {
    const unsigned short* sa = dww_lds + st * PM_DWL_STAGE;
    const unsigned short* sb = sa + 2 * PM_DWL_F * PM_DWW_LDK;
    f32x4 ah[2], al[2];
#pragma unroll
    for (int i = 0; i < 2; ++i) {
      const int tr = (i == 0 || two) ? wid + 8 * i : wid;
      const unsigned short* q = sa + (tr * 16 + c16) * PM_DWW_LDK + g * 8;
      ah[i] = *reinterpret_cast<const f32x4*>(q);
      al[i] = *reinterpret_cast<const f32x4*>(q + PM_DWL_F * PM_DWW_LDK);
    }
#pragma unroll
    for (int j = 0; j < PM_DWL_NT; ++j) {
      const unsigned short* q = sb + (j * 16 + c16) * PM_DWW_LDK + g * 8;
      const f32x4 bh = *reinterpret_cast<const f32x4*>(q);
      const f32x4 bl = *reinterpret_cast<const f32x4*>(q + PM_DWL_F * PM_DWW_LDK);
      acc[0][j] = pm_mfma_bf<false>(al[0], bh, acc[0][j]);
      if (two) acc[1][j] = pm_mfma_bf<false>(al[1], bh, acc[1][j]);
      acc[0][j] = pm_mfma_bf<false>(ah[0], bl, acc[0][j]);
      if (two) acc[1][j] = pm_mfma_bf<false>(ah[1], bl, acc[1][j]);
      acc[0][j] = pm_mfma_bf<false>(ah[0], bh, acc[0][j]);
      if (two) acc[1][j] = pm_mfma_bf<false>(ah[1], bh, acc[1][j]);
    }
  };
  if constexpr (ST == 1) {
    int t = st_steps - 1, k = k_lo;
    fetch(t * A.chunks_per_step + k, k + 1 < k_hi, t);
    stage(0, t * A.chunks_per_step + k, k + 1 < k_hi);
    __syncthreads();
    for (int st = 0;; st ^= 1) {
      int tn = t, kn = k + 2;
      if (kn >= k_hi) { kn = k_lo; tn = t - 1; }
      const bool more = tn >= A.st_cut;
      if (more) fetch(tn * A.chunks_per_step + kn, kn + 1 < k_hi, tn);
      mfmas(st);
      if (more) stage(st ^ 1, tn * A.chunks_per_step + kn, kn + 1 < k_hi);
      __syncthreads();
      if (!more) break;
      t = tn; k = kn;
    }
  } else {
    fetch(R.c_lo, R.c_lo + 1 < R.c_hi, 0);
    stage(0);
    __syncthreads();
    int st = 0;
    for (int c = R.c_lo; c < R.c_hi; c += 2, st ^= 1) {
      const bool more = c + 2 < R.c_hi;
      if (more) fetch(c + 2, c + 3 < R.c_hi, 0);
      mfmas(st);
      if (more) stage(st ^ 1);
      __syncthreads();
    }
  }
  {
    constexpr int LDE = PM_DWL_F + 4;
    float* ep = reinterpret_cast<float*>(dww_lds);
    float* wpart = part + A.w_off[l];
    const bool vec4 = (K & 3) == 0 && (A.w_off[l] & 3) == 0;
    __syncthreads();
#pragma unroll
    for (int half = 0; half < 2; ++half) {
      const int tr0 = 7 * half;
#pragma unroll
      for (int i = 0; i < 2; ++i) {
        const int tr = wid + 8 * i;
        if ((i == 0 || two) && (half == 0 ? tr < 7 : tr >= 7)) {
#pragma unroll
          for (int j = 0; j < PM_DWL_NT; ++j)
#pragma unroll
            for (int r = 0; r < 4; ++r) ep[((tr - tr0) * 16 + 4 * g + r) * LDE + j * 16 + c16] = acc[i][j][r];
        }
      }
      __syncthreads();
      const int o0 = tr0 * 16, nro = min(half == 0 ? 7 * 16 : 6 * 16, max(0, O - o0));
      if (vec4) {
        const int K4 = K >> 2;
        for (int e = tid; e < nro * K4; e += PM_DW_NT) {
          const int ro = e / K4, kq = e - ro * K4;
          const f32x4 v = *reinterpret_cast<const f32x4*>(ep + ro * LDE + 4 * kq);
          f32x4* q = reinterpret_cast<f32x4*>(wpart + (size_t)(o0 + ro) * K + 4 * kq);
          *q = R.add ? *q + v : v;
        }
      } else {
        for (int e = tid; e < nro * K; e += PM_DW_NT) {
          const int ro = e / K, k = e - ro * K;
          pm_dw_put(wpart + (size_t)(o0 + ro) * K + k, ep[ro * LDE + k], R.add);
        }
      }
      __syncthreads();
    }
  }
  if constexpr (ST == 1) {
    if (A.st_head) {
      const int O2 = A.dim[l + 2];
#pragma unroll
      for (int i = 0; i < 2; ++i) {
        const f32x4 v = *reinterpret_cast<const f32x4*>(hd_acc + lane * 12 + 4 * i);
        const int k = (wid + 8 * i) * 16 + c16;
        if (i == 0 || wid + 8 < A.nt[l + 1]) {
#pragma unroll
          for (int r = 0; r < 4; ++r)
            if (4 * g + r < O2 && k < O) part[A.w_off[l + 1] + (size_t)(4 * g + r) * O + k] = v[r];
        }
      }
      float b = hd_acc[lane * 12 + 8];
      b += __shfl_xor(b, 16);
      b += __shfl_xor(b, 32);
      if (wid == 0 && g == 0 && c16 < O2) part[A.b_off[l + 1] + c16] = b;
    }
  }
  if constexpr (RC) {
    rc.bias_out(part + A.b_off[l], O, lane, R.add);
  } else {
#pragma unroll
    for (int j = 0; j < PM_DWL_Q; ++j) {
      float v = cl.bs[j];
      v += __shfl_xor(v, 1);
      v += __shfl_xor(v, 2);
      v += __shfl_xor(v, 4);
      const int idx = tid + PM_DW_NT * j, o = idx >> 3;
      if ((idx & 7) == 0 && o < O) pm_dw_put(part + A.b_off[l] + o, v, R.add);
    }
  }
}
#undef PM_DWL_RT
#undef PM_DWL_RW
__global__ __launch_bounds__(PM_DW_NT, 2) void pm_dw_layer_kernel(const DwArgs A, int l) { pm_dw_layer_body<false>(A, l); }
__global__ __launch_bounds__(PM_DW_NT, 2) void pm_dw_layer_rc_kernel(const DwArgs A, int l) { pm_dw_layer_body<true>(A, l); }
__global__ __launch_bounds__(PM_DW_NT, 2) void pm_dw_layer_st_kernel(const DwArgs A, int l) { pm_dw_layer_body<true, 1>(A, l); }
__global__ __launch_bounds__(PM_DW_NT, 2) void pm_dw_layer_rcb_kernel(const DwArgs A, int l) { pm_dw_layer_body<true, 2>(A, l); }
```

prob_mbrl_amd/csrc/pmbrl_dw_plan.h:

```cpp
#pragma once
#include <algorithm>
#include <cassert>
#include <utility>
#include <vector>

#include "pmbrl_dw.h"

typedef struct ihipStream_t* hipStream_t;
typedef struct ihipEvent_t* hipEvent_t;

#define PM_PIPE_MAX 8
#define PM_REG_DW_LAYER 1

struct DwSwitches {
  bool dw_no_wide;
  bool dw_pipe_off, dw_pipe_ranges;
  std::vector<int> dw_pipe;
  int dw_head;
  bool dw_stream_off, dw_stream_set;
  int dw_stream_steps, dw_stream_wgs;
};

struct DwShape {
  int nl, nt[PM_MAXL + 1], dim[PM_MAXL + 1];
  int w_off[PM_MAXL], b_off[PM_MAXL], n_params;
  int dyn_n_params;
  int prec, RT, fast, inplace, nwg, H, U, cus;
  bool whole;
  int mm_parts, reg, reg_mm;
  bool reg_bwd;
  DwSwitches sw;
};

enum class DwKernel : int {
  None,
  Block, BlockSplit,
  BlockRing,
  NarrowPre1, NarrowPre2,
  Wide, WidePre,
  Layer
};

struct DwPlan {
  DwArgs args;
  std::vector<DwBlock> blocks, blocks_nh;
  bool skip[PM_MAXL];
  DwBlock* blocks_nh_d;
  int wave_first_nh[PM_DW_NW + 1], nh_ring;
  DwKernel table_k, table_nh_k;
  std::vector<DwUnit> units;
  DwUnit* units_d;
  DwKernel unit_k;
  int narrow[PM_MAXL];
  unsigned pre_mask;
  DwKernel layer_k[PM_MAXL];
  int layer13;
  int pipe_K, pipe_lo[PM_PIPE_MAX], pipe_rows, pipe_grid;
  hipStream_t pipe_stream;
  hipEvent_t pipe_ev[PM_PIPE_MAX];
  int st_on, st_cut, st_wgs, st_head;
  size_t off_pub, pub_bytes;
  const void* pub_ws;
  mutable unsigned pub_gen;
  int part_rows;
  size_t off_part;
  int n_blocks() const { return args.wave_first[PM_DW_NW]; }
};

static inline int pm_dw_idle_cus(int cus, int nwg) { return cus >= 64 && cus % 8 == 0 ? 8 * (cus / 8 - (nwg + 7) / 8) : 0; }

inline int build_dw_blocks(int nl, const int* nt, std::vector<DwBlock>& blocks, int* wave_first, int tn_max = PM_DW_TN,
                           const bool* skip = nullptr, int ot_parts_min = 1) {
  blocks.clear();
  auto split = [](int n, int maxsz, std::vector<std::pair<int, int>>& out, int parts_min = 1) {
    const int parts = std::max((n + maxsz - 1) / maxsz, std::min(n, parts_min));
    int lo = 0;
    for (int i = 0; i < parts; ++i) {
      const int sz = n / parts + (i < n % parts ? 1 : 0);
      out.push_back({lo, sz});
      lo += sz;
    }
  };
  for (int l = 0; l < nl; ++l) {
    if (skip && skip[l]) continue;
    std::vector<std::pair<int, int>> os, is;
    split(nt[l + 1], PM_DW_TM, os, ot_parts_min);
    split(nt[l], tn_max, is);
    for (auto& o : os)
      for (auto& i : is)
        blocks.push_back(DwBlock{(int16_t)l, (int16_t)o.first, (int16_t)i.first, (int16_t)o.second, (int16_t)i.second, 0});
  }
  const int n_blocks = (int)blocks.size();
  auto cost = [tn_max](const DwBlock& b) {
    const int ni = b.n_ot <= 1 ? 1 : (b.n_ot <= 3 ? 3 : 4);
    const int nj = b.n_it <= 1 ? 1 : (b.n_it <= 4 ? 4 : (b.n_it <= 6 ? 6 : 7));
    return ni * (tn_max <= 4 && nj > 1 ? 4 : nj);
  };
  std::stable_sort(blocks.begin(), blocks.end(),
                   [&](const DwBlock& a, const DwBlock& b) { return cost(a) > cost(b); });
  std::vector<DwBlock> per_wave[PM_DW_NW];
  long wave_load[PM_DW_NW] = {0};
  for (const DwBlock& b : blocks) {
    int best_simd = 0;
    for (int sm = 1; sm < 4; ++sm)
      if (wave_load[sm] + wave_load[sm + 4] < wave_load[best_simd] + wave_load[best_simd + 4]) best_simd = sm;
    const int w = wave_load[best_simd] <= wave_load[best_simd + 4] ? best_simd : best_simd + 4;
    per_wave[w].push_back(b);
    wave_load[w] += cost(b);
  }
  blocks.clear();
  for (int w = 0; w < PM_DW_NW; ++w) {
    wave_first[w] = (int)blocks.size();
    if (w >= 4) std::reverse(per_wave[w].begin(), per_wave[w].end());
    for (const DwBlock& b : per_wave[w]) blocks.push_back(b);
  }
  wave_first[PM_DW_NW] = (int)blocks.size();
  return n_blocks;
}

inline void pm_dw_plan_blocks(const DwShape& S, DwPlan& P) {
  DwArgs& W = P.args;
  W.split_prec = S.prec != 0 && (S.RT >= 2 || !S.fast);
  bool* wide = P.skip;
  std::vector<DwUnit>& units = P.units;
  P.layer13 = -1;
  if (S.prec != 0 && !S.sw.dw_no_wide)
    for (int l = 0; l < S.nl; ++l)
      if (S.nt[l + 1] * 16 >= 128 && S.nt[l] * 16 >= 128) {
        wide[l] = true;
        if (P.layer13 < 0 && S.nt[l + 1] <= PM_DWL_NT && S.nt[l] <= PM_DWL_NT) {
          P.layer13 = l;
          continue;
        }
        for (int m0 = 0; m0 < S.nt[l + 1] * 16; m0 += PM_DWW_TM)
          for (int n0 = 0; n0 < S.nt[l] * 16; n0 += PM_DWW_TN) units.push_back(DwUnit{(int16_t)l, (int16_t)m0, (int16_t)n0, 0});
      }
  P.unit_k = units.empty() ? DwKernel::None : DwKernel::Wide;
  if (!units.empty() && S.inplace == 2 && S.RT == 4) {
    bool all = true;
    for (const DwUnit& u : units) all = all && S.nt[u.layer] == 32 && S.nt[u.layer + 1] == 32 &&
                                        S.dim[u.layer] == 512 && S.dim[u.layer + 1] == 512;
    for (int l = 0; l < S.nl && all; ++l) {
      bool is = false;
// ... 13 lines not shown
          for (int n0 = 0; n0 < 512; n0 += PM_DWP_TN) pre.push_back(DwUnit{(int16_t)l, (int16_t)m0, (int16_t)n0, 0});
      }
      units = pre;
      P.unit_k = DwKernel::WidePre;
      assert(W.split_prec);
    } else {
      for (int l = 0; l < PM_MAXL; ++l) P.narrow[l] = 0;
    }
  }
  build_dw_blocks(S.nl, S.nt, P.blocks, W.wave_first, W.split_prec ? PM_DW_TN_S : PM_DW_TN, wide);
  P.table_k = P.blocks.empty() ? DwKernel::None : (W.split_prec ? DwKernel::BlockSplit : DwKernel::Block);
  for (int l = 0; l < S.nl; ++l) {
    const int nt_n = P.narrow[l] == 1 ? S.nt[l] : S.nt[l + 1];
    P.layer_k[l] = P.narrow[l]      ? (nt_n <= 1 ? DwKernel::NarrowPre1 : DwKernel::NarrowPre2)
                   : l == P.layer13 ? DwKernel::Layer
                   : wide[l]        ? P.unit_k
                                    : P.table_k;
  }
  W.n_chunks = S.H * S.nwg * S.RT;
  int nsplit = std::min(256, W.n_chunks);
  W.chunks_per_split = (W.n_chunks + nsplit - 1) / nsplit;
  if (W.split_prec) W.chunks_per_split = (W.chunks_per_split + 1) & ~1;
  W.nsplit = (W.n_chunks + W.chunks_per_split - 1) / W.chunks_per_split;
  W.nl = S.nl;
  W.RT = S.RT;
  W.Rw = 16 * S.RT;
  W.n_params = S.n_params;
  W.part_stride = (W.n_params + 3) / 4 * 4;
  for (int i = 0; i <= S.nl; ++i) { W.dim[i] = S.dim[i]; W.nt[i] = S.nt[i]; }
  for (int l = 0; l < S.nl; ++l) { W.w_off[l] = S.w_off[l]; W.b_off[l] = S.b_off[l]; }
  W.chunks_per_step = S.nwg * S.RT;
}

inline void pm_dw_plan_pipe(const DwShape& S, DwPlan& P, int n_free) {
  const DwSwitches& sw = S.sw;
  const int H = S.H, cus = S.cus;
  P.pipe_K = 1;
  const bool no_pipe_pre = P.pre_mask != 0;
  const bool single = S.whole && S.mm_parts <= 1;
  const bool long_steps = (long long)S.RT * (long long)(S.n_params + S.dyn_n_params) >= 256 * 1024 && H >= 16;
  if (!single || no_pipe_pre || n_free < cus / 8 || H < 2 || sw.dw_pipe_off || !(long_steps || sw.dw_pipe_ranges))
    return;
  std::vector<int> cnt;
  if (sw.dw_pipe_ranges) {
    cnt = sw.dw_pipe;
    int sum = 0;
    for (int v : cnt) sum += v;
    if (sum != H || (int)cnt.size() > PM_PIPE_MAX) cnt.clear();
  }
  if (cnt.empty() && long_steps) {
    const int a3 = std::max(2, H / 10), a2 = a3 + std::max(2, H / 5), a1 = a2 + std::max(2, (3 * H) / 10);
    cnt = {H - a1, a1 - a2, a2 - a3, a3};
  }
  int K = 0, lo = H;
  for (size_t k = 0; k < cnt.size() && lo > 0; ++k) {
    lo = k + 1 == cnt.size() ? 0 : std::max(0, lo - cnt[k]);
    if (P.args.split_prec && ((S.nwg * S.RT) & 1) && (lo & 1)) lo -= 1;
    if (K > 0 && lo >= P.pipe_lo[K - 1]) continue;
    P.pipe_lo[K++] = lo;
  }
  if (K >= 2 && P.pipe_lo[K - 1] == 0) {
    P.pipe_K = K;
    P.pipe_grid = n_free;
    P.pipe_rows = std::max(n_free, cus);
  }
}

inline void pm_dw_plan_stream(const DwShape& S, DwPlan& P, int n_free) {
  const DwSwitches& sw = S.sw;
  const int H = S.H, cus = S.cus;
  P.st_on = 0;
  const bool fam = S.reg && !S.reg_mm && S.reg_bwd && P.layer13 == PM_REG_DW_LAYER && S.RT == 1;
  const bool single = S.whole && S.mm_parts <= 1 && P.pipe_K <= 1;
  if (!fam || !single || n_free < 1 || n_free < cus / 8 || sw.dw_stream_off || H >= 4095) return;
  const bool large = S.nwg >= n_free && (long long)H * S.nwg >= 14ll * cus;
  if (!large && !sw.dw_stream_set) return;
  int steps = S.nwg <= 2 * n_free ? H : (int)((long long)H * 2 * n_free / S.nwg);
  int wgs = n_free;
  if (sw.dw_stream_set) {
    steps = sw.dw_stream_steps;
    if (sw.dw_stream_wgs > 0) wgs = std::min(wgs, sw.dw_stream_wgs);
  }
  steps = std::max(0, std::min(H, steps));
  P.st_on = 1;
  P.st_cut = H - steps;
  P.st_wgs = wgs;
}

inline void pm_dw_plan_head(const DwShape& S, DwPlan& P) {
  const DwSwitches& sw = S.sw;
  const DwArgs& W = P.args;
  const int l = P.layer13, h = l + 1;
  P.st_head = 0;
  if (!P.st_on || P.st_cut != 0 || sw.dw_head == 0 || (sw.dw_head < 0 && sw.dw_stream_set)) return;
  if (h != S.nl - 1 || S.nt[h + 1] != 1 || S.dim[h + 1] > 16 || P.skip[h] || W.split_prec) return;
  if (W.b_off[l] != W.w_off[l] + W.dim[l + 1] * W.dim[l] || W.w_off[h] != W.b_off[l] + W.dim[l + 1] ||
      W.b_off[h] != W.w_off[h] + W.dim[h + 1] * W.dim[h])
    return;
  bool skip[PM_MAXL];
  for (int i = 0; i < PM_MAXL; ++i) skip[i] = P.skip[i] || i == h;
  build_dw_blocks(S.nl, S.nt, P.blocks_nh, P.wave_first_nh, PM_DW_TN, skip, PM_DW_NW);
  P.nh_ring = 1;
  for (const DwBlock& b : P.blocks_nh) P.nh_ring = P.nh_ring && b.n_ot <= 2 && b.n_it <= 1;
  P.table_nh_k = P.blocks_nh.empty() ? DwKernel::None : (P.nh_ring ? DwKernel::BlockRing : DwKernel::Block);
  P.st_head = 1;
  assert(P.pipe_K <= 1);
}

inline void pm_dw_plan(const DwShape& S, DwPlan& P) {
  P = DwPlan();
  const int n_free = pm_dw_idle_cus(S.cus, S.nwg);
  pm_dw_plan_blocks(S, P);
  pm_dw_plan_pipe(S, P, n_free);
  pm_dw_plan_stream(S, P, n_free);
  pm_dw_plan_head(S, P);
  P.part_rows = std::max(P.args.nsplit, P.pipe_K > 1 ? P.pipe_rows : 0);
  P.pub_bytes = P.st_on ? (size_t)S.H * S.nwg * 2 * S.U * 16 * sizeof(unsigned long long) : 0;
}
```

prob_mbrl_amd/csrc/pmbrl_host.h:

```cpp
#pragma once
#include <hip/hip_runtime.h>

#include <cmath>
#include <string>
#include <vector>

#include "pmbrl.h"
#include "pmbrl_dev.h"
#include "pmbrl_dw.h"
#include "pmbrl_dw_plan.h"
#include "pmbrl_instances.h"

int pm_fail(int code, const std::string& msg);
static inline int fail(int code, const std::string& msg) { return pm_fail(code, msg); }
#define HIPCHK(expr)                                                               \
  do {                                                                             \
    hipError_t _e = (expr);                                                        \
    if (_e != hipSuccess)                                                          \
      return pm_fail(-100 - (int)_e, std::string(#expr) + ": " + hipGetErrorString(_e)); \
  } while (0)

struct NetPlan {
  int nl;
  int dim[PM_MAXL + 1], nt[PM_MAXL + 1];
// ... 72 lines not shown
  long long* prof_fwd;
  long long* prof_bwd;
  int timing;
  hipEvent_t ev[PMBRL_TIMER_COUNT][2];
  bool ev_set[PMBRL_TIMER_COUNT];
};

enum class SweepForm {
  Barrier,
  StepInSweep,
  Whole,
  StepExternal
};
static inline SweepForm sweep_form(const pmbrl_plan* p) {
  if (p->mm_mode == 3) return p->mm_grid ? SweepForm::Barrier : SweepForm::StepInSweep;
  return p->mm_mode == 2 ? SweepForm::StepExternal : SweepForm::Whole;
}

static inline void replay_drop(pmbrl_plan* p, int slot) {
  if (p->rp[slot].exec) (void)hipGraphExecDestroy(p->rp[slot].exec);
  p->rp[slot].exec = nullptr;
  p->rp[slot].seen = 0;
}

struct ScopedTimer {
  pmbrl_plan* p; int slot; hipStream_t s;
  ScopedTimer(pmbrl_plan* p_, int slot_, hipStream_t s_) : p(p_), slot(slot_), s(s_) {
    if (p->timing) (void)hipEventRecord(p->ev[slot][0], s);
  }
  ~ScopedTimer() {
    if (p->timing) { (void)hipEventRecord(p->ev[slot][1], s); p->ev_set[slot] = true; }
  }
};

static inline std::string pm_inst_name(const PmInstKey& k) {
  std::string s;
  for (int v : {k.rt, k.ca, k.cb, k.var, k.d, k.u, k.ld, k.nl, k.nt, k.tree}) s += (s.empty() ? "(" : ", ") + std::to_string(v);
  return s + ") [row tiles, stage pair, variant, D, U, LD, layers, hidden tiles, tree]";
}

static inline int hidden_tiles_3l(const pmbrl_plan* p) {
  if (p->pol.nl != 3 || p->dyn.nl != 3) return -1;
  const int nt = p->pol.nt[1];
  return p->pol.nt[2] == nt && p->dyn.nt[1] == nt && p->dyn.nt[2] == nt ? nt : -1;
}
static inline int fast_variant(int RT, const RolloutArgs& A) {
  const bool mm = A.mm_mode == 1 || A.mm_mode == 3;
  const bool ext = A.prof || A.grad_states || A.grad_actions || A.agn || A.zpol_ss != 0 || A.zdyn_ss != 0 ||
                   (A.flags & PMBRL_FLAG_MM_STATES) || A.t0 != 0 || A.t1 != A.H || A.gx_from_carry;
  const bool mmg = RT == 1 && A.mm_mode == 3 && A.mm_grid;
  return mmg ? PF_VAR_MMG : mm ? PF_VAR_MM : (ext ? PF_VAR_EXT : PF_VAR_LEAN);
}

struct PackJob {
  const float* src;
  float* dst;
  int O, K, transpose, mult, is_bias;
  int planes;
  int f16;
};
struct PackArgs {
  int n;
  int* wflag;
  int gen;
  int* status;
  PackJob job[6 * PM_MAXL];
};
void pm_pack_all_launch(const PackArgs& PK, hipStream_t s);

int pm_dw_plan_create(pmbrl_plan* p, int cus);
void pm_dw_plan_destroy(pmbrl_plan* p);
hipError_t pm_dw_upload_blocks(const std::vector<DwBlock>& blocks, DwBlock** out);
void pm_dw_bind_blocks(DwArgs& W, const DwBlock* blocks_d, const int* wave_first);
DwArgs pm_dw_call_args(const pmbrl_plan* p, void* workspace, int32_t* status, const RolloutArgs& A, bool rebuilt, bool streamed);
void pm_dw_launch(const pmbrl_plan* p, const DwArgs& W, hipStream_t s, hipEvent_t after = nullptr);
void pm_dw_stream_launch(const pmbrl_plan* p, const DwArgs& W, hipStream_t s);
void pm_dw_launch_range(const pmbrl_plan* p, const DwArgs& W, int k, hipStream_t s);
void pm_dw_blocks_launch(const DwArgs& W, hipStream_t s);
#define PM_NORM_MAXB 8192
void pm_dw_reduce_launch(hipStream_t s, const float* part, int nsplit, int n, int stride, float* grad,
                         const int* nvalid = nullptr, int chunks_per_step = 0, int chunks_per_split = 1, int norm_on = 0,
                         const int* status = nullptr, int expect = 0, long long* step = nullptr, const float* loss_r = nullptr,
                         const float* loss_w = nullptr, long long loss_n = 0, long long loss_per_step = 0, int col_lo = 0,
                         int col_hi = 0, int rows_in_range = 0);
void launch_weighted_sum(hipStream_t s, const float* a, const float* w, long long n, float* out, const int* nvalid,
                         long long n_per_step);
struct AdamStep {
  float *params, *grads, *exp_avg, *exp_avg_sq;
  int64_t n;
  int64_t step = 0;
  int64_t* step_d = nullptr;
  const int32_t* status = nullptr;
  int32_t expect = 0;
  double max_norm = 0.0;
  float* norm_out = nullptr;
  float* loss_out = nullptr;
  int n_loss_part = 0;
  bool norm_done = false;
  double lr = 0.0, beta1 = 0.0, beta2 = 0.0, eps = 0.0;
  const pmbrl_opt_rule* rule = nullptr;
};
int pm_adam_launch(hipStream_t s, const AdamStep& A);
struct OptGroupConsts {
  float wd;
  float decay;
  float sgn;
  int ams;
  double ln_b1, ln_b2;
};
inline OptGroupConsts pm_opt_group_consts(const pmbrl_opt_group& G) {
  const bool dec = G.flags & PMBRL_OPT_DECOUPLED;
  return {dec ? 0.f : (float)G.weight_decay, dec ? (float)(1.0 - G.lr * G.weight_decay) : 1.f,
          (G.flags & PMBRL_OPT_MAXIMIZE) ? -1.f : 1.f, (G.flags & PMBRL_OPT_AMSGRAD) ? 1 : 0, log(G.beta1), log(G.beta2)};
}
const char* pm_act_refusal(int32_t act, int n_hidden);
inline int pm_act_layers(int32_t act, int n_hidden) {
  if (act & PMBRL_ACT_PER_LAYER) return act & ~PMBRL_ACT_PER_LAYER;
  int v = 0;
  for (int l = 0; l < n_hidden; ++l) v |= PMBRL_ACT_LAYER(act, l);
  return v;
}
const char* pm_opt_rule_refusal(const pmbrl_opt_rule* r, int64_t n);
void pm_tail_hvec_launch(hipStream_t s, float* hvec, int world, int rank, const int* status, int H);
void pm_tail_hmin_launch(hipStream_t s, const float* hvec, int world, int* status, int H);
void pm_tail_pack_launch(hipStream_t s, float* xb, int n, int n_loss_part, int loss_here, const int* status, const int* err);
void pm_tail_finish_launch(hipStream_t s, const float* xb, float* g, long long n, int* status, int expect, long long* step,
                           const int* err);
void pm_p2p_describe(const pmbrl_p2p* p, int* rank, int* nranks, size_t* cap_bytes, int** err_d);
bool pm_reg_plan_ok(const pmbrl_plan* p);
bool pm_reg_shape_ok(const pmbrl_plan* p, int prec1);
bool pm_reg_mm_shape_ok(const pmbrl_plan* p, int prec1);
int pm_reg_mm_width(const pmbrl_plan* p);
size_t pm_reg_pack_bytes();
int pm_reg_resolve(pmbrl_plan* p);
bool pm_reg_can_run(const pmbrl_plan* p, const RolloutArgs& A, bool fwd);
struct ZtabArgs;
void pm_reg_pack_launch(const pmbrl_plan* p, char* ws, const float* pol_params, const float* dyn_params, int* wflag, int gen,
                        hipStream_t s, int* status_reset, const ZtabArgs* ztab);
void pm_reg_unpack_abits(const pmbrl_plan* p, char* ws, hipStream_t s);
void pm_reg_dw_rebuild_args(const pmbrl_plan* p, char* ws, DwArgs& W);
void pm_reg_launch(const pmbrl_plan* p, char* ws, const RolloutArgs& A, const float* pol_params, const float* dyn_params,
                   hipStream_t s, bool fwd, unsigned pub = 0, unsigned pub_tag = 0);
PmInstTable pm_fast_f32_instances();
PmInstTable pm_fast_split1_instances();
PmInstTable pm_fast_split2_instances();
PmInstTable pm_general_split_instances();
PmInstTable pm_general_act_instances();
PmInstTable pm_general_gmmr_instances();
PmInstTable pm_general_gmmr_act_instances();
```

prob_mbrl_amd/csrc/pmbrl_tail.hip:

```cpp
#include <hip/hip_runtime.h>
#include <math.h>

#include <algorithm>
#include <string>
#include <type_traits>

#include "pmbrl_host.h"

__global__ void pm_pack_mask_kernel(const float* __restrict__ m, int B, int h, int ld,
                                    uint16_t* __restrict__ bits) {
  const int nt = (h + 15) / 16;
  const int i = blockIdx.x * blockDim.x + threadIdx.x;
  if (i >= B * nt) return;
  const int r = i / nt, t = i - r * nt;
  unsigned w = 0;
  for (int j = 0; j < 16; ++j) {
    const int f = t * 16 + j;
    if (f < h && m[(size_t)r * ld + f] != 0.f) w |= 1u << j;
  }
  bits[i] = (uint16_t)w;
}
__global__ void pm_set_int(int* p, int v) { *p = v; }

struct DrawArgs {
// ... 46 lines not shown
        if (A.u_out) A.u_out[o] = u;
        if (A.hard_out) A.hard_out[o] = bit ? 1.f : 0.f;
        if (A.probs_out) A.probs_out[o] = probs;
      }
    }
  }
  A.bits[i] = (uint16_t)w;
}

#define PM_RED_MAXB 128
__device__ double g_red_part[2][PM_RED_MAXB];
__device__ unsigned g_red_count;

__global__ __launch_bounds__(256) void pm_weighted_sum_kernel(const float* __restrict__ a,
                                                              const float* __restrict__ w,
                                                              long long n, float* __restrict__ out,
                                                              const int* __restrict__ nvalid, long long n_per_step) {
  __shared__ double sm[256];
  __shared__ unsigned ticket;
  if (nvalid) n = min(n, (long long)max(0, *nvalid) * n_per_step);
  double s = 0.0;
  const long long stride = (long long)gridDim.x * blockDim.x;
  for (long long i = (long long)blockIdx.x * blockDim.x + threadIdx.x; i < n; i += 8 * stride) {
    float av[8], wv[8];
#pragma unroll
    for (int u = 0; u < 8; ++u) {
      const long long j = min(i + u * stride, n - 1);
      av[u] = a[j];
      wv[u] = w[j];
    }
#pragma unroll
    for (int u = 0; u < 8; ++u) s += i + u * stride < n ? (double)av[u] * (double)wv[u] : 0.0;
  }
  const double tot = pm_block_sum(s, sm);
  if (threadIdx.x == 0) {
    __hip_atomic_store(&g_red_part[0][blockIdx.x], tot, __ATOMIC_RELAXED, __HIP_MEMORY_SCOPE_AGENT);
    asm volatile("s_waitcnt vmcnt(0)" ::: "memory");
    ticket = __hip_atomic_fetch_add(&g_red_count, 1u, __ATOMIC_RELAXED, __HIP_MEMORY_SCOPE_AGENT);
  }
  __syncthreads();
  if (ticket == gridDim.x - 1) {
    __builtin_amdgcn_fence(__ATOMIC_ACQUIRE, "agent");
    double t = 0.0;
    for (unsigned b = threadIdx.x; b < gridDim.x; b += blockDim.x)
      t += __hip_atomic_load(&g_red_part[0][b], __ATOMIC_RELAXED, __HIP_MEMORY_SCOPE_AGENT);
    __syncthreads();
    const double tt = pm_block_sum(t, sm);
    if (threadIdx.x == 0) {
      out[0] = (float)tt;
      __hip_atomic_store(&g_red_count, 0u, __ATOMIC_RELAXED, __HIP_MEMORY_SCOPE_AGENT);
    }
  }
}

__device__ double g_norm_part[PM_NORM_MAXB];
__device__ double g_loss_part[PM_NORM_MAXB];
__device__ int g_adam_go;
__device__ __forceinline__ double pm_sq4_wave(const f32x4& t, long long i0, long long n) {
  double s = 0.0;
#pragma unroll
  for (int r = 0; r < 4; ++r) {
    const double x = i0 + r < n ? (double)t[r] : 0.0;
    s += x * x;
  }
#pragma unroll
  for (int o = 32; o > 0; o >>= 1) s += __shfl_xor(s, o);
  return s;
}
__device__ __forceinline__ void pm_adam_decide(const int* status, int expect, long long* step) {
  const int go = (!status || (status[0] >= expect && status[1] == 0)) ? 1 : 0;
  g_adam_go = go;
  if (go && step) step[0] += 1;
}

__global__ __launch_bounds__(512) void pm_dw_reduce(const float* __restrict__ part, int nsplit, int n,
                                                    int stride, float* __restrict__ grad,
                                                    const int* __restrict__ nvalid = nullptr, int chunks_per_step = 0,
                                                    int chunks_per_split = 1, int norm_on = 0,
                                                    const int* __restrict__ status = nullptr, int expect = 0,
                                                    long long* __restrict__ step = nullptr,
                                                    const float* __restrict__ loss_r = nullptr,
                                                    const float* __restrict__ loss_w = nullptr, long long loss_n = 0,
                                                    long long loss_per_step = 0, int col_lo = 0, int col_hi = 0,
                                                    int rows_in_range = 0) {
  __shared__ f32x4 sm[8][64];
  __shared__ double sl_[8];
  float lr4[4] = {0.f, 0.f, 0.f, 0.f}, lw4[4] = {0.f, 0.f, 0.f, 0.f};
  long long l_n = 0;
  const long long l_i0 = (long long)blockIdx.x * blockDim.x + threadIdx.x, l_st = (long long)gridDim.x * blockDim.x;
  if (loss_r) {
    l_n = nvalid ? min(loss_n, (long long)max(0, *nvalid) * loss_per_step) : loss_n;
#pragma unroll
    for (int u = 0; u < 4; ++u) {
      const long long j = min(l_i0 + u * l_st, loss_n - 1);
      lr4[u] = loss_r[j];
      lw4[u] = loss_w[j];
    }
  }
  if (nvalid) {
    const long long nc = (long long)max(0, *nvalid) * chunks_per_step;
    nsplit = (int)min((long long)nsplit, (nc + chunks_per_split - 1) / chunks_per_split);
  }
  const int col = threadIdx.x & 63, sl = threadIdx.x >> 6;
  const int c4 = blockIdx.x * 64 + col;
  const int per = (nsplit + 7) / 8;
  int k_hi = min(nsplit, sl * per + per);
  const int k_lo = sl * per;
  if (c4 * 4 >= col_lo && c4 * 4 + 4 <= col_hi) k_hi = min(k_hi, rows_in_range);
  f32x4 s = f32x4{0.f, 0.f, 0.f, 0.f};
  if (c4 * 4 < n) {
    const float* p = part + (size_t)c4 * 4;
    int k = k_lo;
    for (; k + 16 <= k_hi; k += 16) {
      f32x4 v[16];
#pragma unroll
      for (int u = 0; u < 16; ++u) v[u] = ldg4(p + (size_t)(k + u) * stride);
#pragma unroll
      for (int u = 0; u < 16; ++u) s += v[u];
    }
    for (; k < k_hi; k += 8) {
      f32x4 v[8];
#pragma unroll
      for (int u = 0; u < 8; ++u) v[u] = ldg4(p + (size_t)min(k + u, k_hi - 1) * stride);
#pragma unroll
      for (int u = 0; u < 8; ++u) s += k + u < k_hi ? v[u] : f32x4{0.f, 0.f, 0.f, 0.f};
    }
  }
  sm[sl][col] = s;
  if (loss_r) {
    double ls = 0.0;
#pragma unroll
    for (int u = 0; u < 4; ++u) ls += l_i0 + u * l_st < l_n ? (double)lr4[u] * (double)lw4[u] : 0.0;
    for (long long j = l_i0 + 4 * l_st; j < l_n; j += l_st) ls += (double)loss_r[j] * (double)loss_w[j];
#pragma unroll
    for (int o = 32; o > 0; o >>= 1) ls += __shfl_xor(ls, o);
    if (col == 0) sl_[sl] = ls;
  }
  __syncthreads();
  if (loss_r && threadIdx.x == 0) {
    double t = sl_[0];
#pragma unroll
    for (int k = 1; k < 8; ++k) t += sl_[k];
    g_loss_part[blockIdx.x] = t;
  }
  if (sl == 0) {
    f32x4 t = f32x4{0.f, 0.f, 0.f, 0.f};
    if (c4 * 4 < n) {
      t = sm[0][col];
#pragma unroll
      for (int k = 1; k < 8; ++k) t += sm[k][col];
#pragma unroll
      for (int r = 0; r < 4; ++r)
        if (c4 * 4 + r < n) grad[c4 * 4 + r] = t[r];
    }
    if (norm_on) {
      const double s2 = pm_sq4_wave(t, (long long)c4 * 4, n);
      if (col == 0) {
        g_norm_part[blockIdx.x] = s2;
        if (blockIdx.x == 0) pm_adam_decide(status, expect, step);
      }
    }
  }
}

static inline int pm_norm_blocks(long long n) { return (int)std::max<long long>(1, std::min<long long>(PM_NORM_MAXB, (n + 255) / 256)); }
template <bool COPY>
__device__ __forceinline__ void pm_norm_walk(const float* __restrict__ src, float* __restrict__ dst, long long n) {
  double tot = 0.0;
  for (long long eb = blockIdx.x; eb * 256 < n; eb += gridDim.x) {
    const long long i0 = eb * 256 + 4 * (long long)threadIdx.x;
    f32x4 t = f32x4{0.f, 0.f, 0.f, 0.f};
    if (i0 + 3 < n) {
      t = *reinterpret_cast<const f32x4*>(src + i0);
      if constexpr (COPY)
        for (int r = 0; r < 4; ++r) dst[i0 + r] = t[r];
    } else {
      for (int r = 0; r < 4; ++r) {
        t[r] = i0 + r < n ? src[i0 + r] : 0.f;
        if constexpr (COPY)
          if (i0 + r < n) dst[i0 + r] = t[r];
      }
    }
    tot += pm_sq4_wave(t, i0, n);
  }
  if (threadIdx.x == 0) g_norm_part[blockIdx.x] = tot;
}
__global__ __launch_bounds__(64) void pm_gradnorm_kernel(const float* __restrict__ g, long long n,
                                                         const int* __restrict__ status, int expect,
                                                         long long* __restrict__ step, int guarded) {
  if (guarded && blockIdx.x == 0 && threadIdx.x == 0) pm_adam_decide(status, expect, step);
  pm_norm_walk<false>(g, nullptr, n);
}

__device__ __forceinline__ void pm_norm_request(double (&part)[4], int lane, int n_part) {
#pragma unroll
  for (int u = 0; u < 4; ++u) {
    const double x = g_norm_part[min(lane + 64 * u, PM_NORM_MAXB - 1)];
    part[u] = lane + 64 * u < n_part ? x : 0.0;
  }
}
__device__ __forceinline__ double pm_norm_sum(const double (&part)[4], int lane, int n_part) {
  double t = 0.0;
#pragma unroll
  for (int u = 0; u < 4; ++u) t += part[u];
  for (int b = lane + 256; b < n_part; b += 64) t += g_norm_part[b];
#pragma unroll
  for (int o = 32; o > 0; o >>= 1) t += __shfl_xor(t, o);
  return t;
// ... 230 lines not shown
  D.vmax = ams ? r.max_exp_avg_sq_d : nullptr;
  return D;
}

void launch_weighted_sum(hipStream_t s, const float* a, const float* w, long long n, float* out, const int* nvalid,
                                long long n_per_step) {
  const int nb = (int)std::max<long long>(1, std::min<long long>(PM_RED_MAXB, (n + 2047) / 2048));
  hipLaunchKernelGGL(pm_weighted_sum_kernel, dim3(nb), dim3(256), 0, s, a, w, n, out, nvalid, n_per_step);
}

int pm_adam_launch(hipStream_t s, const AdamStep& A) {
  const int guarded = A.step_d ? 1 : 0;
  const int nb = (int)std::max<long long>(1, std::min<long long>(PM_RED_MAXB, (A.n + 1023) / 1024));
  const int np = pm_norm_blocks(A.n);
  const bool need_norm = guarded ? !A.norm_done : (A.max_norm > 0.0 || A.norm_out != nullptr);
  long long* const step_d = reinterpret_cast<long long*>(A.step_d);
  if (need_norm)
    hipLaunchKernelGGL(pm_gradnorm_kernel, dim3(np), dim3(64), 0, s, A.grads, (long long)A.n, (const int*)A.status,
                       (int)A.expect, step_d, guarded);
  const int n_part = guarded || need_norm ? np : 0;
  auto launch = [&](const auto& R) {
    hipLaunchKernelGGL(pm_clip_adam_kernel<std::decay_t<decltype(R)>>, dim3(nb), dim3(256), 0, s, A.params, A.grads, A.exp_avg,
                       A.exp_avg_sq, (long long)A.n, n_part, (float)A.max_norm, A.norm_out, (const long long*)step_d, guarded,
                       A.loss_out, A.n_loss_part, R);
  };
  if (A.rule) {
    const OptRuleDev D = opt_rule_dev(*A.rule, guarded ? 0 : (long long)A.step);
    if (D.vmax) launch(AdamTable<true>{D});
    else launch(AdamTable<false>{D});
  } else {
    AdamPlain P;
    P.b1 = (float)A.beta1; P.b2 = (float)A.beta2;
    P.omb1 = (float)(1.0 - A.beta1); P.omb2 = (float)(1.0 - A.beta2);
    P.eps = (float)A.eps;
    P.bc1 = P.bc2_sqrt = 1.f;
    if (!guarded) {
      P.bc1 = (float)(1.0 - pow(A.beta1, (double)A.step));
      P.bc2_sqrt = (float)sqrt(1.0 - pow(A.beta2, (double)A.step));
    }
    P.ln_b1 = log(A.beta1); P.ln_b2 = log(A.beta2); P.lr_d = A.lr;
    launch(P);
  }
  HIPCHK(hipGetLastError());
  return 0;
}

__global__ __launch_bounds__(64) void pm_tail_hvec_kernel(float* __restrict__ hvec, int world, int rank,
                                                          const int* __restrict__ status, int H) {
  for (int q = threadIdx.x; q < world; q += blockDim.x) hvec[q] = q == rank ? (float)min(max(status[0], 0), H) : 0.f;
}
__global__ __launch_bounds__(64) void pm_tail_hmin_kernel(const float* __restrict__ hvec, int world,
                                                          int* __restrict__ status, int H) {
  if (threadIdx.x != 0) return;
  int m = H;
  for (int q = 0; q < world; ++q) m = min(m, (int)hvec[q]);
  if (m < min(status[0], H)) status[0] = m;
}
__global__ __launch_bounds__(64) void pm_tail_pack_kernel(float* __restrict__ xb, int n, int n_loss_part, int loss_here,
                                                          const int* __restrict__ status, const int* __restrict__ err) {
  const int lane = threadIdx.x;
  if (n_loss_part > 0) {
    const double ls = pm_loss_sum(lane, n_loss_part);
    if (lane == 0) xb[n] = (float)ls;
  } else if (!loss_here && lane == 0) {
    xb[n] = 0.f;
  }
  if (lane == 0) xb[n + 1] = (status[1] != 0 || (err && *err != 0)) ? 1.f : 0.f;
}
__global__ __launch_bounds__(64) void pm_tail_finish_kernel(const float* __restrict__ xb, float* __restrict__ g, long long n,
                                                            int* __restrict__ status, int expect,
                                                            long long* __restrict__ step, const int* __restrict__ err) {
  if (blockIdx.x == 0 && threadIdx.x == 0) {
    const int bad = (xb[n + 1] != 0.f || (err && *err != 0)) ? 1 : 0;
    if (bad) status[1] = 1;
    pm_adam_decide(status, expect, step);
    g_loss_part[0] = (double)xb[n];
  }
  pm_norm_walk<true>(xb, g, n);
}

void pm_dw_reduce_launch(hipStream_t s, const float* part, int nsplit, int n, int stride, float* grad, const int* nvalid,
                         int chunks_per_step, int chunks_per_split, int norm_on, const int* status, int expect, long long* step,
                         const float* loss_r, const float* loss_w, long long loss_n, long long loss_per_step, int col_lo,
                         int col_hi, int rows_in_range) {
  hipLaunchKernelGGL(pm_dw_reduce, dim3((n + 255) / 256), dim3(512), 0, s, part, nsplit, n, stride, grad, nvalid,
                     chunks_per_step, chunks_per_split, norm_on, status, expect, step, loss_r, loss_w, loss_n, loss_per_step,
                     col_lo, col_hi, rows_in_range);
}
void pm_tail_hvec_launch(hipStream_t s, float* hvec, int world, int rank, const int* status, int H) {
  hipLaunchKernelGGL(pm_tail_hvec_kernel, dim3(1), dim3(64), 0, s, hvec, world, rank, status, H);
}
void pm_tail_hmin_launch(hipStream_t s, const float* hvec, int world, int* status, int H) {
  hipLaunchKernelGGL(pm_tail_hmin_kernel, dim3(1), dim3(64), 0, s, hvec, world, status, H);
}
void pm_tail_pack_launch(hipStream_t s, float* xb, int n, int n_loss_part, int loss_here, const int* status, const int* err) {
  hipLaunchKernelGGL(pm_tail_pack_kernel, dim3(1), dim3(64), 0, s, xb, n, n_loss_part, loss_here, status, err);
}
void pm_tail_finish_launch(hipStream_t s, const float* xb, float* g, long long n, int* status, int expect, long long* step,
                           const int* err) {
  hipLaunchKernelGGL(pm_tail_finish_kernel, dim3(pm_norm_blocks(n)), dim3(64), 0, s, xb, g, n, status, expect, step, err);
}

extern "C" int pmbrl_pack_mask(void* stream, const float* mask_d, int32_t B, int32_t h,
                               int32_t src_ld, uint16_t* bits_d) {
  if (!mask_d || !bits_d || B < 1 || h < 1 || src_ld < h) return fail(-1, "bad argument");
  const int nt = (h + 15) / 16;
  const int n = B * nt;
  hipLaunchKernelGGL(pm_pack_mask_kernel, dim3((n + 255) / 256), dim3(256), 0, (hipStream_t)stream,
                     mask_d, B, h, src_ld, bits_d);
  HIPCHK(hipGetLastError());
  return 0;
}

extern "C" int pmbrl_draw_masks(void* stream, int32_t kind, uint64_t seed, uint64_t offset, const float* param_d,
                                int32_t param_len, float temp, int32_t rows, int32_t h, const float* u_d, const float* v_d,
                                uint16_t* bits_d, int32_t aux_row0, int32_t aux_rows, float* u_out_d, float* hard_out_d,
                                float* probs_out_d) {
  if (!param_d || !bits_d || rows < 1 || h < 1 || (kind != 0 && kind != 1) || (param_len != 1 && param_len != h) ||
      aux_row0 < 0 || aux_rows < 0 || aux_row0 + aux_rows > rows)
    return fail(-1, "bad argument");
  if (kind == 1 && !(temp > 0.f)) return fail(-1, "concrete dropout needs a positive temperature");
  DrawArgs A;
  A.kind = kind; A.seed = seed; A.offset = offset; A.param = param_d; A.param_len = param_len; A.temp = temp;
  A.rows = rows; A.h = h; A.u_in = u_d; A.v_in = v_d; A.bits = bits_d;
  A.aux_row0 = aux_row0; A.aux_rows = aux_rows; A.u_out = u_out_d; A.hard_out = hard_out_d; A.probs_out = probs_out_d;
  const long long n = (long long)rows * ((h + 15) / 16);
  hipLaunchKernelGGL(pm_draw_masks_kernel, dim3((unsigned)((n + 255) / 256)), dim3(256), 0, (hipStream_t)stream, A);
  HIPCHK(hipGetLastError());
  return 0;
}

extern "C" int pmbrl_weighted_sum(void* stream, const float* a_d, const float* w_d, int64_t n,
                                  float* out_d) {
  if (!a_d || !w_d || !out_d || n < 0) return fail(-1, "bad argument");
  launch_weighted_sum((hipStream_t)stream, a_d, w_d, n, out_d, nullptr, 0);
  HIPCHK(hipGetLastError());
  return 0;
}

extern "C" int pmbrl_weighted_sum_steps(void* stream, const float* a_d, const float* w_d, int64_t n_per_step,
                                        int32_t n_steps, const int32_t* status_d, float* out_d) {
  if (!a_d || !w_d || !out_d || n_per_step < 0 || n_steps < 0) return fail(-1, "bad argument");
  launch_weighted_sum((hipStream_t)stream, a_d, w_d, (long long)n_per_step * n_steps, out_d, status_d, n_per_step);
  HIPCHK(hipGetLastError());
  return 0;
}

static AdamStep adam_step_on(float* params_d, float* grads_d, float* exp_avg_d, float* exp_avg_sq_d, int64_t n, double max_norm,
                             float* norm_out_d) {
  AdamStep A;
  A.params = params_d; A.grads = grads_d; A.exp_avg = exp_avg_d; A.exp_avg_sq = exp_avg_sq_d; A.n = n;
  A.max_norm = max_norm; A.norm_out = norm_out_d;
  return A;
}
extern "C" int pmbrl_clip_adam(void* stream, float* params_d, float* grads_d, float* exp_avg_d,
                               float* exp_avg_sq_d, int64_t n, int64_t step, double lr, double beta1,
                               double beta2, double eps, double max_norm, float* norm_out_d) {
  if (!params_d || !grads_d || !exp_avg_d || !exp_avg_sq_d || n < 1 || step < 1)
    return fail(-1, "bad argument");
  AdamStep A = adam_step_on(params_d, grads_d, exp_avg_d, exp_avg_sq_d, n, max_norm, norm_out_d);
  A.step = step;
  A.lr = lr; A.beta1 = beta1; A.beta2 = beta2; A.eps = eps;
  return pm_adam_launch((hipStream_t)stream, A);
}

extern "C" int pmbrl_clip_adam_guarded(void* stream, float* params_d, float* grads_d, float* exp_avg_d,
                                       float* exp_avg_sq_d, int64_t n, int64_t* step_d, double lr,
                                       double beta1, double beta2, double eps, double max_norm,
                                       float* norm_out_d, const int32_t* status_d, int32_t expect) {
  if (!params_d || !grads_d || !exp_avg_d || !exp_avg_sq_d || !step_d || !status_d || n < 1)
// ... 30 lines not shown
```

prob_mbrl_amd/engine.py:

```python
import ctypes as C
import math

import numpy as np
import torch

from . import _lib

LOG_MAX_STD = math.log(5.0)

_PRECISIONS = {'f32': _lib.PREC_F32, 'split': _lib.PREC_SPLIT, 'split_f16': _lib.PREC_SPLIT_F16}
_default_precision = [None]


def set_precision(name):
    assert name in _PRECISIONS, name
    _default_precision[0] = name


def get_precision():
    import os
    return _default_precision[0] or os.environ.get('PMBRL_PRECISION', 'split_f16')


def safe_precision(name):
# ... 605 lines not shown

    def backward(self, grad_rewards, grad_states=None, grad_actions=None, want_x0=False,
                 want_agn=False, adam=None):
        assert self._inputs is not None, 'forward() first'
        dev = self.device
        gr = _f32c(grad_rewards.reshape(self.H, self.B), dev)
        gs = _f32c(grad_states, dev) if grad_states is not None else None
        ga = _f32c(grad_actions, dev) if grad_actions is not None else None
        if gs is not None:
            assert gs.shape == (self.H + 1, self.B, self.D)
        if ga is not None:
            assert ga.shape == (self.H, self.B, self.U)
        gx0 = torch.empty((self.B, self.D), dtype=torch.float32, device=dev) if want_x0 else None
        agn = torch.empty((self.H, self.B), dtype=torch.float32, device=dev) if want_agn else None
        S, A, R = self._traj
        if adam is not None:
            for k in ('params', 'exp_avg', 'exp_avg_sq'):
                t = adam[k]
                assert t.is_cuda and t.dtype == torch.float32 and t.is_contiguous() and t.numel() == self.n_pol_params
            assert adam['step'].is_cuda and adam['step'].dtype == torch.int64
            self.set_optimizer(adam.get('rule'))
            o = _lib.Adam(adam['params'].data_ptr(), adam['exp_avg'].data_ptr(), adam['exp_avg_sq'].data_ptr(),
                          adam['step'].data_ptr(), float(adam['lr']), float(adam['betas'][0]), float(adam['betas'][1]),
                          float(adam['eps']), float(adam.get('max_norm') or 0.0),
                          adam['norm_out'].data_ptr() if adam.get('norm_out') is not None else None,
                          int(adam.get('expect') or 0),
                          adam['loss_out'].data_ptr() if adam.get('loss_out') is not None else None)
            if adam.get('loss_out') is not None:
                lo = adam['loss_out']
                assert lo.is_cuda and lo.dtype == torch.float32 and lo.numel() >= 1
            _lib.check(self.lib.pmbrl_rollout_bwd_adam(self.plan, _stream(), self._ws_ptr,
                                                       C.byref(self._inputs), _ptr(S), _ptr(A), _ptr(R), _ptr(gr),
                                                       _ptr(gs), _ptr(ga), _ptr(self.grad_flat), _ptr(gx0),
                                                       _ptr(agn), _ptr(self.status), C.byref(o)),
                       'pmbrl_rollout_bwd_adam')
            return self.grad_flat, gx0, agn
        _lib.check(self.lib.pmbrl_rollout_bwd(self.plan, _stream(), self._ws_ptr,
                                              C.byref(self._inputs), _ptr(S), _ptr(A), _ptr(R), _ptr(gr),
                                              _ptr(gs), _ptr(ga), _ptr(self.grad_flat), _ptr(gx0),
                                              _ptr(agn), _ptr(self.status)),
                   'pmbrl_rollout_bwd')
        return self.grad_flat, gx0, agn

    def set_optimizer(self, rule):
        _attach_rule(self, 'pmbrl_plan_set_optimizer', rule, self.n_pol_params)

    def set_replay(self, on=1):
        _lib.check(self.lib.pmbrl_plan_set_replay(self.plan, int(on)), 'set_replay')
        info = (C.c_int32 * _lib.INFO_COUNT)()
        _lib.check(self.lib.pmbrl_plan_info(self.plan, info), 'plan_info')
        self.info['replay'] = int(info[_lib.INFO_REPLAY])

    def reg_calls(self):
        info = (C.c_int32 * _lib.INFO_COUNT)()
        _lib.check(self.lib.pmbrl_plan_info(self.plan, info), 'plan_info')
        return int(info[_lib.INFO_REG_FWD_CALLS]), int(info[_lib.INFO_REG_BWD_CALLS])

    def sweep_kernels(self):
        out = {}
        for v, key in enumerate(_lib.SWEEP_VARIANTS):
            if key in ('ext', 'mm', 'mmg') and not self.info['fast']:
                continue
            names = []
            for adjoint in (0, 1):
                name = C.c_char_p()
                _lib.check(self.lib.pmbrl_plan_sweep_kernel(self.plan, v, adjoint, C.byref(name)), 'plan_sweep_kernel')
                names.append((name.value or b'').decode())
            if names[0]:
                out[key] = tuple(names)
        return out

    def dw_stream(self):
        if not hasattr(self.lib, 'pmbrl_plan_dw_stream'):
            return None
        out = (C.c_int32 * 2)()
        _lib.check(self.lib.pmbrl_plan_dw_stream(self.plan, out), 'plan_dw_stream')
        return None if out[0] < 0 else (int(out[0]), int(out[1]))

    def dw_head(self):
        if not hasattr(self.lib, 'pmbrl_plan_dw_head'):
            return False
        return bool(self.lib.pmbrl_plan_dw_head(self.plan))

    def replay_count(self):
        n = (C.c_int64 * 2)()
        _lib.check(self.lib.pmbrl_plan_replay_count(self.plan, n), 'replay_count')
        return int(n[0]), int(n[1])

    def set_timing(self, on=True):
        _lib.check(self.lib.pmbrl_plan_set_timing(self.plan, 1 if on else 0), 'set_timing')

    def read_timing(self):
        ms = (C.c_float * _lib.TIMER_COUNT)()
        _lib.check(self.lib.pmbrl_plan_read_timing(self.plan, ms), 'read_timing')
        return {n: float(ms[i]) for i, n in enumerate(_lib.TIMER_NAMES)}

    def weighted_sum(self, a, w, out=None):
        a = _f32c(a.reshape(-1), self.device)
        w = _f32c(w.reshape(-1), self.device)
        assert a.numel() == self.H * self.B and w.numel() == a.numel()
        if out is None:
            out = torch.empty(1, dtype=torch.float32, device=self.device)
        _lib.check(self.lib.pmbrl_weighted_sum_steps(_stream(), _ptr(a), _ptr(w), self.B, self.H,
                                                     _ptr(self.status), _ptr(out)),
                   'pmbrl_weighted_sum_steps')
        return out


def _rule_struct(rule, n):
    if rule.vmax is not None:
        v = rule.vmax
        assert v.is_cuda and v.dtype == torch.float32 and v.is_contiguous() and v.numel() == n
    return rule.struct()


def _attach_rule(owner, setter, rule, n):
    if rule is None and not getattr(owner, '_has_rule', False):
        return
    r = _rule_struct(rule, n) if rule is not None else None
    _lib.check(getattr(owner.lib, setter)(owner.plan, C.byref(r) if r is not None else None), setter)
    owner._has_rule = rule is not None


def _clip_adam(name, params, grads, exp_avg, exp_avg_sq, step, guard, lr, betas, eps, max_norm, norm_out, rule):
    lib = _lib.load()
    for t in (params, grads, exp_avg, exp_avg_sq):
        assert t.is_cuda and t.dtype == torch.float32 and t.is_contiguous()
    n = params.numel()
    head = (_stream(), _ptr(params), _ptr(grads), _ptr(exp_avg), _ptr(exp_avg_sq), n, step)
    tail = (float(max_norm) if max_norm else 0.0, _ptr(norm_out)) + guard
    if rule is not None:
        name = name.replace('clip_adam', 'clip_adam_rule')
        r = _rule_struct(rule, n)
        _lib.check(getattr(lib, name)(*head, *tail, C.byref(r)), name)
        return
    _lib.check(getattr(lib, name)(*head, float(lr), float(betas[0]), float(betas[1]), float(eps), *tail), name)


def clip_adam(params, grads, exp_avg, exp_avg_sq, step, lr=None, betas=(0.9, 0.999), eps=1e-8,
              max_norm=None, norm_out=None, rule=None):
    _clip_adam('pmbrl_clip_adam', params, grads, exp_avg, exp_avg_sq, int(step), (), lr, betas, eps, max_norm, norm_out, rule)


class Graph:

    def __init__(self, fn, warmup=1):
        self.lib = _lib.load()
        self.handle = C.c_void_p()
        side = torch.cuda.Stream()
        side.wait_stream(torch.cuda.current_stream())
        with torch.cuda.stream(side):
            for _ in range(warmup):
                fn()
            side.synchronize()
            _lib.check(self.lib.pmbrl_graph_capture_begin(C.c_void_p(side.cuda_stream)), 'pmbrl_graph_capture_begin')
            try:
                fn()
            finally:
                rc = self.lib.pmbrl_graph_capture_end(C.c_void_p(side.cuda_stream), C.byref(self.handle))
            _lib.check(rc, 'pmbrl_graph_capture_end')
        torch.cuda.current_stream().wait_stream(side)
        self._keep = fn

    def replay(self):
        _lib.check(self.lib.pmbrl_graph_launch(self.handle, _stream()), 'pmbrl_graph_launch')

# ... 33 lines not shown
```

Before: 6.439 million.

## Rotate streamed dW chunk assignment per step and shrink head block grid to free CUs

```diff
diff --git a/include/pmbrl.h b/include/pmbrl.h
--- a/include/pmbrl.h
+++ b/include/pmbrl.h
@@ -134,6 +134,8 @@
 int pmbrl_plan_sweep_kernel(const pmbrl_plan* plan, int variant, int adjoint, const char** name);
 int pmbrl_plan_dw_stream(const pmbrl_plan* plan, int32_t* out );
 int pmbrl_plan_dw_head(const pmbrl_plan* plan);
+int pmbrl_plan_dw_deal(const pmbrl_plan* plan, int32_t* out );
+int pmbrl_plan_dw_prof(const pmbrl_plan* plan, uint64_t* out, int64_t n);
 
 int pmbrl_pack_mask(void* stream, const float* mask_d, int32_t B, int32_t h,
                     int32_t src_ld, uint16_t* bits_d);
diff --git a/prob_mbrl_amd/_lib.py b/prob_mbrl_amd/_lib.py
--- a/prob_mbrl_amd/_lib.py
+++ b/prob_mbrl_amd/_lib.py
@@ -90,7 +90,7 @@
     'pmbrl_last_error', 'pmbrl_version', 'pmbrl_build_id', 'pmbrl_plan_create',
     'pmbrl_graph_capture_begin', 'pmbrl_graph_capture_end', 'pmbrl_graph_launch', 'pmbrl_graph_num_nodes', 'pmbrl_graph_destroy',
     'pmbrl_plan_destroy', 'pmbrl_plan_workspace_bytes', 'pmbrl_plan_info', 'pmbrl_plan_sweep_kernel', 'pmbrl_plan_dw_stream',
-    'pmbrl_plan_dw_head',
+    'pmbrl_plan_dw_head', 'pmbrl_plan_dw_deal', 'pmbrl_plan_dw_prof',
     'pmbrl_pack_mask', 'pmbrl_draw_masks', 'pmbrl_rollout_fwd', 'pmbrl_rollout_bwd', 'pmbrl_rollout_bwd_adam',
     'pmbrl_plan_set_loss',
     'pmbrl_weighted_sum', 'pmbrl_weighted_sum_steps', 'pmbrl_clip_adam', 'pmbrl_clip_adam_guarded', 'pmbrl_debug_linear',
@@ -174,6 +174,11 @@
     if hasattr(lib, 'pmbrl_plan_dw_head'):
         lib.pmbrl_plan_dw_head.restype = C.c_int
         lib.pmbrl_plan_dw_head.argtypes = [vp]
+    if hasattr(lib, 'pmbrl_plan_dw_deal'):
+        lib.pmbrl_plan_dw_deal.restype = C.c_int
+        lib.pmbrl_plan_dw_deal.argtypes = [vp, C.POINTER(i32)]
+        lib.pmbrl_plan_dw_prof.restype = C.c_int
+        lib.pmbrl_plan_dw_prof.argtypes = [vp, C.POINTER(C.c_uint64), i64]
     lib.pmbrl_pack_mask.restype = C.c_int
     lib.pmbrl_pack_mask.argtypes = [vp, vp, i32, i32, i32, vp]
     lib.pmbrl_rollout_fwd.restype = C.c_int
diff --git a/prob_mbrl_amd/csrc/pmbrl.hip b/prob_mbrl_amd/csrc/pmbrl.hip
--- a/prob_mbrl_amd/csrc/pmbrl.hip
+++ b/prob_mbrl_amd/csrc/pmbrl.hip
@@ -399,6 +399,9 @@
       if (const char* q = strchr(e, ',')) s.dw_stream_wgs = std::max(0, atoi(q + 1));
     }
   }
+  if (const char* e = getenv("PMBRL_DW_DEAL")) s.dw_deal_fixed = !strcmp(e, "fixed");
+  if (const char* e = getenv("PMBRL_DW_BLOCK_ROWS")) { s.dw_block_rows_all = !strcmp(e, "all"); s.dw_block_rows_free = !strcmp(e, "free"); }
+  s.dw_prof = env_set("PMBRL_DW_PROF");
   return s;
 }
 
@@ -1099,6 +1102,22 @@
 }
 
 extern "C" int pmbrl_plan_dw_head(const pmbrl_plan* p) { return p && p->dw.st_on && p->dw.st_head ? 1 : 0; }
+
+extern "C" int pmbrl_plan_dw_deal(const pmbrl_plan* p, int32_t* out) {
+  if (!p || !out) return fail(-1, "null argument");
+  out[0] = p->dw.st_on ? p->dw.st_q : 0;
+  out[1] = p->dw.st_on && p->dw.st_head ? p->dw.nh_rows : 0;
+  return 0;
+}
+
+extern "C" int pmbrl_plan_dw_prof(const pmbrl_plan* p, uint64_t* out, int64_t n) {
+  if (!p || !out) return fail(-1, "null argument");
+  const int64_t need = (int64_t)p->dw.st_wgs * p->cfg.H * 2;
+  if (!p->dw.st_prof_d || n < need) return fail(-1, "no stamps (PMBRL_DW_PROF), or out too small");
+  HIPCHK(hipSetDevice(p->device));
+  HIPCHK(hipMemcpy(out, p->dw.st_prof_d, (size_t)need * sizeof(uint64_t), hipMemcpyDeviceToHost));
+  return 0;
+}
 
 extern "C" int pmbrl_plan_info(const pmbrl_plan* p, int32_t* info) {
   if (!p || !info) return fail(-1, "null argument");
@@ -1795,7 +1814,7 @@
                           W.chunks_per_split, norm_fused ? 1 : 0, (const int*)C.status, expect,
                           opt ? reinterpret_cast<long long*>(opt->step_d) : (long long*)nullptr,
                           loss_fused ? C.rewards : (const float*)nullptr, C.grad_rewards, (long long)p->cfg.H * p->cfg.B,
-                          (long long)p->cfg.B, W.own_lo, W.own_hi, W.st_wgs);
+                          (long long)p->cfg.B, W.own_lo, W.own_hi, W.st_wgs, W.st_head ? p->dw.nh_rows : 0, p->dw.nh_cps);
   }
   if (opt && opt->loss_out_d && !loss_fused)
     launch_weighted_sum(s, C.rewards, C.grad_rewards, (long long)p->cfg.H * p->cfg.B, tail ? xb + n : opt->loss_out_d, C.status,
@@ -1853,6 +1872,10 @@
   K.val(streamed);
   const int head = streamed && p->dw.st_head ? 1 : 0;
   K.val(head);
+  const int deal_q = streamed ? p->dw.st_q : 0;
+  K.val(deal_q);
+  const int block_rows = head ? p->dw.nh_rows : 0;
+  K.val(block_rows);
   return K;
 }
 
diff --git a/prob_mbrl_amd/csrc/pmbrl_dw.h b/prob_mbrl_amd/csrc/pmbrl_dw.h
--- a/prob_mbrl_amd/csrc/pmbrl_dw.h
+++ b/prob_mbrl_amd/csrc/pmbrl_dw.h
@@ -53,8 +53,43 @@
   int* st_fail;
   int own_lo, own_hi;
   int st_head;
+  int st_q, st_H;
+  unsigned long long* st_prof;
 };
-static_assert(sizeof(DwArgs) == 472, "DwArgs is a kernel argument: its layout does not move");
+static_assert(sizeof(DwArgs) == 488, "DwArgs is a kernel argument: its layout does not move");
+
+#ifdef __HIPCC__
+#define PM_DW_HD __host__ __device__
+#else
+#define PM_DW_HD
+#endif
+struct DwDeal {
+  int n, nc, q;
+  int dq, rq, d1, r1;
+  int i, lo, rem;
+  PM_DW_HD void at(int n_, int nc_, int H, int q_, int w, int t) {
+    n = n_; nc = nc_; q = q_;
+    const unsigned un = (unsigned)n, unc = (unsigned)nc, qn = (unsigned)q * un;
+    dq = (int)(qn / unc); rq = (int)(qn - (unsigned)dq * unc);
+    d1 = (int)(un / unc); r1 = (int)(un - (unsigned)d1 * unc);
+    const unsigned k = (unsigned)w + (unsigned)(H - 1 - t) * (unsigned)q;
+    i = (int)(k - k / unc * unc);
+    const unsigned in = (unsigned)i * un;
+    lo = (int)(in / unc); rem = (int)(in - (unsigned)lo * unc);
+  }
+  PM_DW_HD void down() {
+    i += q; lo += dq; rem += rq;
+    if (rem >= nc) { rem -= nc; lo += 1; }
+    if (i >= nc) { i -= nc; lo -= n; }
+  }
+  PM_DW_HD int hi() const { return lo + d1 + (rem + r1 >= nc ? 1 : 0); }
+};
+PM_DW_HD inline void pm_dw_slice(int n, int nc, int H, int q, int w, int t, int& lo, int& hi) {
+  DwDeal D;
+  D.at(n, nc, H, q, w, t);
+  lo = D.lo;
+  hi = D.hi();
+}
 #define PM_DWH_LDS_BYTES ((2 * 16 * 16 + PM_DW_NW * 64 * 12) * 4)
 
 #define PM_DWP_TM 256
diff --git a/prob_mbrl_amd/csrc/pmbrl_dw.hip b/prob_mbrl_amd/csrc/pmbrl_dw.hip
--- a/prob_mbrl_amd/csrc/pmbrl_dw.hip
+++ b/prob_mbrl_amd/csrc/pmbrl_dw.hip
@@ -13,6 +13,7 @@
       {layer, reinterpret_cast<const void*>(&pm_dw_layer_kernel), PM_DWL_LDS_BYTES},
       {layer, reinterpret_cast<const void*>(&pm_dw_layer_rc_kernel), PM_DWL_LDS_BYTES},
       {layer, reinterpret_cast<const void*>(&pm_dw_layer_st_kernel), PM_DWL_LDS_BYTES + PM_DWH_LDS_BYTES},
+      {layer, reinterpret_cast<const void*>(&pm_dw_layer_stp_kernel), PM_DWL_LDS_BYTES + PM_DWH_LDS_BYTES},
       {layer, reinterpret_cast<const void*>(&pm_dw_layer_rcb_kernel), PM_DWL_LDS_BYTES},
       {pre, reinterpret_cast<const void*>(&pm_dw_narrow_pre_kernel<1>), PM_DWP_LDS_BYTES},
       {pre, reinterpret_cast<const void*>(&pm_dw_narrow_pre_kernel<2>), PM_DWP_LDS_BYTES},
@@ -48,6 +49,11 @@
   S.sw = p->sw;
   DwPlan& D = p->dw;
   pm_dw_plan(S, D);
+  if (D.st_on && p->sw.dw_prof) {
+    const size_t bytes = (size_t)D.st_wgs * S.H * 2 * sizeof(unsigned long long);
+    HIPCHK(hipMalloc(&D.st_prof_d, bytes));
+    HIPCHK(hipMemset(D.st_prof_d, 0, bytes));
+  }
   if (!D.units.empty()) {
     HIPCHK(hipMalloc(&D.units_d, D.units.size() * sizeof(DwUnit)));
     HIPCHK(hipMemcpy(D.units_d, D.units.data(), D.units.size() * sizeof(DwUnit), hipMemcpyHostToDevice));
@@ -73,6 +79,7 @@
   if (D.args.blocks) (void)hipFree(const_cast<DwBlock*>(D.args.blocks));
   if (D.blocks_nh_d) (void)hipFree(D.blocks_nh_d);
   if (D.units_d) (void)hipFree(D.units_d);
+  if (D.st_prof_d) (void)hipFree(D.st_prof_d);
   if (D.pipe_stream) (void)hipStreamDestroy(D.pipe_stream);
   for (int k = 0; k < PM_PIPE_MAX; ++k)
     if (D.pipe_ev[k]) (void)hipEventDestroy(D.pipe_ev[k]);
@@ -88,6 +95,9 @@
     W.st_pub = reinterpret_cast<const unsigned long long*>(static_cast<char*>(workspace) + D.off_pub);
     W.st_tag = ((++D.pub_gen) << 12) + 1u;
     W.st_fail = status ? status + 1 : nullptr;
+    W.st_q = D.st_q;
+    W.st_H = p->cfg.H;
+    W.st_prof = D.st_prof_d;
     if (W.st_cut == 0) {
       const int l = D.layer13;
       if (W.b_off[l] == W.w_off[l] + W.dim[l + 1] * W.dim[l]) {
@@ -129,10 +139,13 @@
   const DwPlan& D = p->dw;
   const int n_units = (int)D.units.size();
   const dim3 rows(W.nsplit), units((W.nsplit + 7) / 8 * 8 * n_units);
+  DwArgs Wt = W;
+  if (W.st_head) { Wt.nsplit = D.nh_rows; Wt.chunks_per_split = D.nh_cps; }
+  const dim3 trows(Wt.nsplit);
   switch (W.st_head ? D.table_nh_k : D.table_k) {
-    case DwKernel::Block: hipLaunchKernelGGL(pm_dw_kernel, rows, dim3(PM_DW_NT), 0, s, W); break;
-    case DwKernel::BlockSplit: hipLaunchKernelGGL(pm_dw_kernel_s, rows, dim3(PM_DW_NT), 0, s, W); break;
-    case DwKernel::BlockRing: hipLaunchKernelGGL(pm_dw_kernel_nh, rows, dim3(PM_DW_NT), 0, s, W); break;
+    case DwKernel::Block: hipLaunchKernelGGL(pm_dw_kernel, trows, dim3(PM_DW_NT), 0, s, Wt); break;
+    case DwKernel::BlockSplit: hipLaunchKernelGGL(pm_dw_kernel_s, trows, dim3(PM_DW_NT), 0, s, Wt); break;
+    case DwKernel::BlockRing: hipLaunchKernelGGL(pm_dw_kernel_nh, trows, dim3(PM_DW_NT), 0, s, Wt); break;
     default: break;
   }
   for (int l = 0; l < W.nl; ++l) {
@@ -156,8 +169,8 @@
 void pm_dw_launch_range(const pmbrl_plan* p, const DwArgs& W, int k, hipStream_t s) { pm_dw_launch(p, dw_range_args(p->dw, W, k, p->cfg.H), s); }
 void pm_dw_stream_launch(const pmbrl_plan* p, const DwArgs& W, hipStream_t s) {
   assert(W.st_on && W.rc_abits);
-  hipLaunchKernelGGL(pm_dw_layer_st_kernel, dim3(W.st_wgs), dim3(PM_DW_NT), PM_DWL_LDS_BYTES + PM_DWH_LDS_BYTES, s, W,
-                     p->dw.layer13);
+  hipLaunchKernelGGL(W.st_prof ? pm_dw_layer_stp_kernel : pm_dw_layer_st_kernel, dim3(W.st_wgs), dim3(PM_DW_NT),
+                     PM_DWL_LDS_BYTES + PM_DWH_LDS_BYTES, s, W, p->dw.layer13);
 }
 void pm_dw_blocks_launch(const DwArgs& W, hipStream_t s) {
   hipLaunchKernelGGL(pm_dw_kernel, dim3(W.nsplit), dim3(PM_DW_NT), 0, s, W);
diff --git a/prob_mbrl_amd/csrc/pmbrl_dw_kernels.h b/prob_mbrl_amd/csrc/pmbrl_dw_kernels.h
--- a/prob_mbrl_amd/csrc/pmbrl_dw_kernels.h
+++ b/prob_mbrl_amd/csrc/pmbrl_dw_kernels.h
@@ -1149,7 +1149,12 @@
 static_assert(PM_DWH_LDS_BYTES == (PM_DWH_TAB + PM_DW_NW * PM_DWH_WAVE) * 4, "the head's LDS");
 #define PM_DWL_RT (ST == 1 ? 1 : A.RT)
 #define PM_DWL_RW (ST == 1 ? 16 : A.Rw)
-template <bool RC, int ST = 0>
+__device__ __forceinline__ unsigned long long pm_dw_stamp() {
+  unsigned long long t;
+  asm volatile("s_memrealtime %0\n\ts_waitcnt lgkmcnt(0)" : "=s"(t)::"memory");
+  return t;
+}
+template <bool RC, int ST = 0, bool PROF = false>
 __device__ __forceinline__ void pm_dw_layer_body(const DwArgs& A, int l) {
   static_assert(RC || ST == 0, "the streamed form rebuilds its operand");
   extern __shared__ __attribute__((aligned(16))) unsigned short dww_lds[];
@@ -1157,13 +1162,18 @@
   const int wid = __builtin_amdgcn_readfirstlane(tid >> 6);
   const int row = blockIdx.x;
   DwRange R;
-  int st_steps = 0, k_lo = 0, k_hi = 0;
+  int st_t = 0, st_nc = 1, k_lo = 0, k_hi = 0;
+  unsigned long long prof_wait = 0;
+  DwDeal deal;
   if constexpr (ST == 1) {
     const DwStream S = pm_dw_stream(A);
     if (!S.any || row >= S.nc) return;
-    st_steps = S.steps;
-    k_lo = (int)((long long)row * A.chunks_per_step / S.nc);
-    k_hi = (int)((long long)(row + 1) * A.chunks_per_step / S.nc);
+    st_nc = S.nc;
+    st_t = S.steps - 1;
+    for (deal.at(A.chunks_per_step, st_nc, A.st_H, A.st_q, row, st_t);; --st_t, deal.down()) {
+      k_lo = deal.lo; k_hi = deal.hi();
+      if (k_lo < k_hi || st_t <= A.st_cut) break;
+    }
     R.add = false;
     R.zero = k_lo >= k_hi;
     R.c_lo = R.c_hi = 0;
@@ -1359,7 +1369,13 @@
     if constexpr (ST == 1) {
       __builtin_amdgcn_sched_barrier(0);
       if (A.st_head) head_load(c, second);
-      rc.settle(A, lane);
+      if constexpr (PROF) {
+        const unsigned long long t0 = pm_dw_stamp();
+        rc.settle(A, lane);
+        prof_wait += pm_dw_stamp() - t0;
+      } else {
+        rc.settle(A, lane);
+      }
       if (A.st_head) head_mfma();
       __builtin_amdgcn_sched_barrier(0);
     }
@@ -1396,20 +1412,41 @@
     }
   };
   if constexpr (ST == 1) {
-    int t = st_steps - 1, k = k_lo;
+    int t = st_t, k = k_lo;
+    int t_dn = t, lo_dn = 0, hi_dn = 0;
+    auto step_down = [&]() {
+      do {
+        if (--t_dn < A.st_cut) break;
+        deal.down();
+        lo_dn = deal.lo; hi_dn = deal.hi();
+      } while (lo_dn >= hi_dn);
+    };
     fetch(t * A.chunks_per_step + k, k + 1 < k_hi, t);
+    step_down();
     stage(0, t * A.chunks_per_step + k, k + 1 < k_hi);
     __syncthreads();
     for (int st = 0;; st ^= 1) {
-      int tn = t, kn = k + 2;
-      if (kn >= k_hi) { kn = k_lo; tn = t - 1; }
+      int tn = t, kn = k + 2, lo_n = k_lo, hi_n = k_hi;
+      const bool cross = kn >= k_hi;
+      if (cross) { tn = t_dn; kn = lo_n = lo_dn; hi_n = hi_dn; }
       const bool more = tn >= A.st_cut;
-      if (more) fetch(tn * A.chunks_per_step + kn, kn + 1 < k_hi, tn);
+      if (more) fetch(tn * A.chunks_per_step + kn, kn + 1 < hi_n, tn);
+      if (cross && more) step_down();
       mfmas(st);
-      if (more) stage(st ^ 1, tn * A.chunks_per_step + kn, kn + 1 < k_hi);
+      if (more) stage(st ^ 1, tn * A.chunks_per_step + kn, kn + 1 < hi_n);
       __syncthreads();
+      if constexpr (PROF) {
+        if (tn != t) {
+          if (tid == 0) {
+            unsigned long long* q = A.st_prof + ((size_t)row * A.st_H + t) * 2;
+            q[0] = pm_dw_stamp();
+            q[1] = prof_wait;
+          }
+          prof_wait = 0;
+        }
+      }
       if (!more) break;
-      t = tn; k = kn;
+      t = tn; k = kn; k_lo = lo_n; k_hi = hi_n;
     }
   } else {
     fetch(R.c_lo, R.c_lo + 1 < R.c_hi, 0);
@@ -1501,3 +1538,4 @@
 __global__ __launch_bounds__(PM_DW_NT, 2) void pm_dw_layer_rc_kernel(const DwArgs A, int l) { pm_dw_layer_body<true>(A, l); }
 __global__ __launch_bounds__(PM_DW_NT, 2) void pm_dw_layer_st_kernel(const DwArgs A, int l) { pm_dw_layer_body<true, 1>(A, l); }
 __global__ __launch_bounds__(PM_DW_NT, 2) void pm_dw_layer_rcb_kernel(const DwArgs A, int l) { pm_dw_layer_body<true, 2>(A, l); }
+__global__ __launch_bounds__(PM_DW_NT, 2) void pm_dw_layer_stp_kernel(const DwArgs A, int l) { pm_dw_layer_body<true, 1, true>(A, l); }
diff --git a/prob_mbrl_amd/csrc/pmbrl_dw_plan.h b/prob_mbrl_amd/csrc/pmbrl_dw_plan.h
--- a/prob_mbrl_amd/csrc/pmbrl_dw_plan.h
+++ b/prob_mbrl_amd/csrc/pmbrl_dw_plan.h
@@ -19,6 +19,9 @@
   int dw_head;
   bool dw_stream_off, dw_stream_set;
   int dw_stream_steps, dw_stream_wgs;
+  bool dw_deal_fixed;
+  bool dw_block_rows_all, dw_block_rows_free;
+  bool dw_prof;
 };
 
 struct DwShape {
@@ -59,6 +62,8 @@
   hipStream_t pipe_stream;
   hipEvent_t pipe_ev[PM_PIPE_MAX];
   int st_on, st_cut, st_wgs, st_head;
+  int st_q, nh_rows, nh_cps;
+  unsigned long long* st_prof_d;
   size_t off_pub, pub_bytes;
   const void* pub_ws;
   mutable unsigned pub_gen;
@@ -238,9 +243,30 @@
     if (sw.dw_stream_wgs > 0) wgs = std::min(wgs, sw.dw_stream_wgs);
   }
   steps = std::max(0, std::min(H, steps));
+  if ((long long)wgs * S.nwg * S.RT >= (1ll << 31)) return;
   P.st_on = 1;
   P.st_cut = H - steps;
   P.st_wgs = wgs;
+}
+
+inline int pm_dw_deal_shift(int n, int nc) {
+  auto size = [&](int i) {
+    int lo, hi;
+    pm_dw_slice(n, nc, 1, 0, i, 0, lo, hi);
+    return hi - lo;
+  };
+  int best_q = 0, best = 0;
+  for (int q = 1; q < nc; ++q) {
+    int worst = 0;
+    for (int i = 0; i < nc; ++i) worst = std::max(worst, size(i) + size((i + q) % nc));
+    if (best_q == 0 || worst < best) { best_q = q; best = worst; }
+  }
+  return best_q;
+}
+inline void pm_dw_plan_deal(const DwShape& S, DwPlan& P) {
+  P.st_q = 0;
+  if (!P.st_on || P.st_cut != 0 || S.sw.dw_deal_fixed) return;
+  P.st_q = pm_dw_deal_shift(S.nwg * S.RT, P.st_wgs);
 }
 
 inline void pm_dw_plan_head(const DwShape& S, DwPlan& P) {
@@ -260,6 +286,14 @@
   for (const DwBlock& b : P.blocks_nh) P.nh_ring = P.nh_ring && b.n_ot <= 2 && b.n_it <= 1;
   P.table_nh_k = P.blocks_nh.empty() ? DwKernel::None : (P.nh_ring ? DwKernel::BlockRing : DwKernel::Block);
   P.st_head = 1;
+  bool covers = true;
+  for (int i = 0; i < S.nl; ++i) covers = covers && (i == l || i == h || !P.skip[i]);
+  const int free_cus = S.cus - P.st_wgs;
+  const bool asked = !sw.dw_block_rows_all && (sw.dw_block_rows_free || !sw.dw_stream_set);
+  if (covers && asked && free_cus >= 1 && free_cus < W.nsplit) {
+    P.nh_cps = (W.n_chunks + free_cus - 1) / free_cus;
+    P.nh_rows = (W.n_chunks + P.nh_cps - 1) / P.nh_cps;
+  }
   assert(P.pipe_K <= 1);
 }
 
@@ -269,6 +303,9 @@
   pm_dw_plan_blocks(S, P);
   pm_dw_plan_pipe(S, P, n_free);
   pm_dw_plan_stream(S, P, n_free);
+  pm_dw_plan_deal(S, P);
+  P.nh_rows = P.args.nsplit;
+  P.nh_cps = P.args.chunks_per_split;
   pm_dw_plan_head(S, P);
   P.part_rows = std::max(P.args.nsplit, P.pipe_K > 1 ? P.pipe_rows : 0);
   P.pub_bytes = P.st_on ? (size_t)S.H * S.nwg * 2 * S.U * 16 * sizeof(unsigned long long) : 0;
diff --git a/prob_mbrl_amd/csrc/pmbrl_host.h b/prob_mbrl_amd/csrc/pmbrl_host.h
--- a/prob_mbrl_amd/csrc/pmbrl_host.h
+++ b/prob_mbrl_amd/csrc/pmbrl_host.h
@@ -178,7 +178,7 @@
                          const int* nvalid = nullptr, int chunks_per_step = 0, int chunks_per_split = 1, int norm_on = 0,
                          const int* status = nullptr, int expect = 0, long long* step = nullptr, const float* loss_r = nullptr,
                          const float* loss_w = nullptr, long long loss_n = 0, long long loss_per_step = 0, int col_lo = 0,
-                         int col_hi = 0, int rows_in_range = 0);
+                         int col_hi = 0, int rows_in_range = 0, int rows_out = 0, int cps_out = 1);
 void launch_weighted_sum(hipStream_t s, const float* a, const float* w, long long n, float* out, const int* nvalid,
                          long long n_per_step);
 struct AdamStep {
diff --git a/prob_mbrl_amd/csrc/pmbrl_tail.hip b/prob_mbrl_amd/csrc/pmbrl_tail.hip
--- a/prob_mbrl_amd/csrc/pmbrl_tail.hip
+++ b/prob_mbrl_amd/csrc/pmbrl_tail.hip
@@ -152,7 +152,7 @@
                                                     const float* __restrict__ loss_r = nullptr,
                                                     const float* __restrict__ loss_w = nullptr, long long loss_n = 0,
                                                     long long loss_per_step = 0, int col_lo = 0, int col_hi = 0,
-                                                    int rows_in_range = 0) {
+                                                    int rows_in_range = 0, int rows_out = 0, int cps_out = 1) {
   __shared__ f32x4 sm[8][64];
   __shared__ double sl_[8];
   float lr4[4] = {0.f, 0.f, 0.f, 0.f}, lw4[4] = {0.f, 0.f, 0.f, 0.f};
@@ -170,15 +170,21 @@
   if (nvalid) {
     const long long nc = (long long)max(0, *nvalid) * chunks_per_step;
     nsplit = (int)min((long long)nsplit, (nc + chunks_per_split - 1) / chunks_per_split);
+    rows_out = (int)min((long long)rows_out, (nc + cps_out - 1) / cps_out);
   }
   const int col = threadIdx.x & 63, sl = threadIdx.x >> 6;
   const int c4 = blockIdx.x * 64 + col;
   const int per = (nsplit + 7) / 8;
   int k_hi = min(nsplit, sl * per + per);
   const int k_lo = sl * per;
-  if (c4 * 4 >= col_lo && c4 * 4 + 4 <= col_hi) k_hi = min(k_hi, rows_in_range);
+  const int e_lo = c4 * 4, e_hi = min(c4 * 4 + 4, n);
+  if (rows_out <= 0 || col_lo >= col_hi) rows_out = nsplit;
+  const bool inside = e_lo >= col_lo && e_hi <= col_hi, outside = e_hi <= col_lo || e_lo >= col_hi;
+  const bool edge = !inside && !outside && rows_out < nsplit;
+  if (inside) k_hi = min(k_hi, rows_in_range);
+  else if (outside) k_hi = min(k_hi, rows_out);
   f32x4 s = f32x4{0.f, 0.f, 0.f, 0.f};
-  if (c4 * 4 < n) {
+  if (c4 * 4 < n && !edge) {
     const float* p = part + (size_t)c4 * 4;
     int k = k_lo;
     for (; k + 16 <= k_hi; k += 16) {
@@ -194,6 +200,20 @@
       for (int u = 0; u < 8; ++u) v[u] = ldg4(p + (size_t)min(k + u, k_hi - 1) * stride);
 #pragma unroll
       for (int u = 0; u < 8; ++u) s += k + u < k_hi ? v[u] : f32x4{0.f, 0.f, 0.f, 0.f};
+    }
+  } else if (c4 * 4 < n) {
+    const float* p = part + (size_t)c4 * 4;
+    for (int k = k_lo; k < k_hi; k += 8) {
+      f32x4 v[8];
+#pragma unroll
+      for (int u = 0; u < 8; ++u) v[u] = ldg4(p + (size_t)min(k + u, k_hi - 1) * stride);
+#pragma unroll
+      for (int u = 0; u < 8; ++u)
+#pragma unroll
+        for (int r = 0; r < 4; ++r) {
+          const bool in = e_lo + r >= col_lo && e_lo + r < col_hi;
+          s[r] += (k + u < k_hi && (in || k + u < rows_out)) ? v[u][r] : 0.f;
+        }
     }
   }
   sm[sl][col] = s;
@@ -590,10 +610,10 @@
 void pm_dw_reduce_launch(hipStream_t s, const float* part, int nsplit, int n, int stride, float* grad, const int* nvalid,
                          int chunks_per_step, int chunks_per_split, int norm_on, const int* status, int expect, long long* step,
                          const float* loss_r, const float* loss_w, long long loss_n, long long loss_per_step, int col_lo,
-                         int col_hi, int rows_in_range) {
+                         int col_hi, int rows_in_range, int rows_out, int cps_out) {
   hipLaunchKernelGGL(pm_dw_reduce, dim3((n + 255) / 256), dim3(512), 0, s, part, nsplit, n, stride, grad, nvalid,
                      chunks_per_step, chunks_per_split, norm_on, status, expect, step, loss_r, loss_w, loss_n, loss_per_step,
-                     col_lo, col_hi, rows_in_range);
+                     col_lo, col_hi, rows_in_range, rows_out, cps_out);
 }
 void pm_tail_hvec_launch(hipStream_t s, float* hvec, int world, int rank, const int* status, int H) {
   hipLaunchKernelGGL(pm_tail_hvec_kernel, dim3(1), dim3(64), 0, s, hvec, world, rank, status, H);
diff --git a/prob_mbrl_amd/engine.py b/prob_mbrl_amd/engine.py
--- a/prob_mbrl_amd/engine.py
+++ b/prob_mbrl_amd/engine.py
@@ -711,6 +711,22 @@
             return False
         return bool(self.lib.pmbrl_plan_dw_head(self.plan))
 
+    def dw_deal(self):
+        if not hasattr(self.lib, 'pmbrl_plan_dw_deal'):
+            return (0, 0)
+        out = (C.c_int32 * 2)()
+        _lib.check(self.lib.pmbrl_plan_dw_deal(self.plan, out), 'plan_dw_deal')
+        return int(out[0]), int(out[1])
+
+    def dw_prof(self):
+        st = self.dw_stream()
+        if st is None:
+            raise RuntimeError('dw_prof: the plan streams nothing')
+        torch.cuda.synchronize()
+        out = np.zeros((st[1], int(self.H), 2), dtype=np.uint64)
+        _lib.check(self.lib.pmbrl_plan_dw_prof(self.plan, out.ctypes.data_as(C.POINTER(C.c_uint64)), out.size), 'plan_dw_prof')
+        return out
+
     def replay_count(self):
         n = (C.c_int64 * 2)()
         _lib.check(self.lib.pmbrl_plan_replay_count(self.plan, n), 'replay_count')
```

Measured after the change: 6.447 million (median of 3 runs). Within noise of the previous version (+0.1%).
